# szbonaldo/FedMLP

Measured on AMD Instinct MI355X. Metric: images/sec/client (ICH 224x224 bs=128) at 1/2/4/8 GPUs; mAP vs ref, higher is better.
Workload: dtype f32; 1 GPU; FedMLP stage1 step, Resnet18, ICH-shaped synthetic 3x224x224, C=5, bs=128, one client per GPU, FedAvg all-reduce every 40 steps + once at end; parallelism=clients1, rccl_ranks=1, stream_mode=default: frozen teacher + weight gradients on the engine's side stream, arithmetic=fp32 operands+sums; products as 6 exact bf16 partials on the bf16 matrix pipe

## Files before the change

### fedmlp_amd/_lib.py

```python
import ctypes as C
import os

_HERE = os.path.dirname(os.path.abspath(__file__))
LIB_PATH = os.environ.get("FEDMLP_HIP_LIB") or os.path.join(_HERE, "libfedmlp_hip.so")

FM_MAX_CLASSES = 32
FM_MAX_GROUPS = 8
FM_COMM_ID_BYTES = 128


class FmConfig(C.Structure):
    _fields_ = [("model", C.c_int32), ("n_classes", C.c_int32), ("in_h", C.c_int32),
                ("in_w", C.c_int32), ("max_images", C.c_int32), ("reserved", C.c_int32 * 3),
                ("stream", C.c_void_p)]


class FmAdam(C.Structure):
    _fields_ = [("lr", C.c_float), ("beta1", C.c_float), ("beta2", C.c_float),
                ("eps", C.c_float), ("weight_decay", C.c_float)]


class FmSgd(C.Structure):
    _fields_ = [("lr", C.c_float), ("momentum", C.c_float), ("dampening", C.c_float),
                ("weight_decay", C.c_float), ("nesterov", C.c_int32)]
# ... 17 lines not shown
    "fm_counters": (C.c_int, [_P, _P, _I32]),
    "fm_state_scale": (C.c_int, [_P, C.c_float]),
    "fm_fedavg_fold": (C.c_int, [_P, C.POINTER(_P), _F, _I32, _P]),
    "fm_fed_w": (C.c_int, [_P, C.POINTER(_P), C.POINTER(C.c_double), _I32, _P]),
    "fm_state_dist": (C.c_int, [_P, C.POINTER(_P), _I32, _P, _P, _I32]),
    "fm_stream_mode": (C.c_int, [_P]),
    "fm_mfma_products": (C.c_int, []),
    "fm_products": (C.c_int, [_P]),
    "fm_planes_mode": (C.c_int, [_P]),
    "fm_teacher_snapshot": (C.c_int, [_P]),
    "fm_adam_reset": (C.c_int, [_P, C.POINTER(FmAdam)]),
    "fm_forward_eval": (C.c_int, [_P, _P, _I32, _I32, _P, _P]),
    "fm_step_bce": (C.c_int, [_P, _P, _P, _I32, _F, _I32, _P]),
    "fm_step_stage1": (C.c_int, [_P, _P, _P, _P, _I32, _F, _I32, _I32, _P]),
    "fm_step_stage2": (C.c_int, [_P, _P, _P, _P, _I32, _P]),
    "fm_step_fixmatch": (C.c_int, [_P, _P, _P, _P, _I32, _F, _F, _F, _I32, _I32, _P]),
    "fm_loss_fedlsr": (C.c_int, [_P, _P, _P, _F, C.c_float, C.c_float, _I32, _P, _P]),
    "fm_loss_fedirm_sup": (C.c_int, [_P, _P, _P, _F, _F, _I32, _I32, _I32, _P, _P, _P]),
    "fm_loss_fedirm_rel": (C.c_int, [_P, _P, _P, _P, _F, _F, _I32, _I32, C.c_float, _P, _I32, _P, _P, _P]),
    "fm_step_fedlsr": (C.c_int, [_P, _P, _P, _P, _I32, _F, C.c_float, C.c_float, _P]),
    "fm_loss_rscfed": (C.c_int, [_P, _P, _P, _P, _F, _F, _I32, _I32, _I32, _P, _P]),
    "fm_loss_lakd": (C.c_int, [_P, _P, _P, _P, _F, C.c_float, _I32, _P, _P]),
    "fm_loss_cbafed": (C.c_int, [_P, _P, _P, _F, _I32, _I32, _F, _I32, _P, _P, _P, _P]),
    "fm_step_rscfed": (C.c_int, [_P, _P, _P, _P, _I32, _F, _F, _I32, _I32, C.c_float, C.c_float, _P]),
    "fm_step_fednoro": (C.c_int, [_P, _P, _P, _I32, _F, C.c_float, _P]),
    "fm_step_cbafed": (C.c_int, [_P, _P, _P, _I32, _F, _I32, _I32, _F, _P, _P, _P]),
    "fm_proto_reset": (C.c_int, [_P]),
    "fm_proto_accumulate": (C.c_int, [_P, _P, _P, _P, _I32, _F, _F, C.c_float, C.c_float]),
    "fm_proto_finalize": (C.c_int, [_P, _I32, _I64, _F, _P, _P]),
    "fm_cos_tag": (C.c_int, [_P, _P, _I64, _P, C.POINTER(_I32), _I32, _P]),
    "fm_select_topk": (C.c_int, [_P, _P, _I64, C.c_double, C.c_double, _I32, C.POINTER(_I32),
                                 C.POINTER(_I32), C.POINTER(_I32), C.POINTER(_I32)]),
    "fm_select_topk_rows": (C.c_int, [_P, _P, _I64, _I32, C.POINTER(_I32), C.POINTER(_I32), _I32, C.c_double, C.c_double, _I32,
                                      C.POINTER(_I32), C.POINTER(_I32), C.POINTER(_I32), C.POINTER(_I32)]),
    "fm_augment": (C.c_int, [_P, _P, _P, _P, _I32, _F, _F, _P]),
    "fm_augment_strong": (C.c_int, [_P, _P, _P, _P, _P, _I32, _F, _F, _P]),
    "fm_eval_metrics": (C.c_int, [_P, _P, _P, _I64, _I32, C.c_float, _P, _P, _P]),
    "fm_forward_train": (C.c_int, [_P, _P, _P, _I32, _P, _P]),
    "fm_backward_step": (C.c_int, [_P, _P]),
    "fm_backward_grads": (C.c_int, [_P, _P, _P]),
    "fm_backward_grads_x": (C.c_int, [_P, _P, _P, _P, _P]),
    "fm_forward_recompute": (C.c_int, [_P, _P, _P, _I32]),
    "fm_zero_grad": (C.c_int, [_P]),
    "fm_adam_step": (C.c_int, [_P, C.POINTER(FmAdam)]),
    "fm_get_grads": (C.c_int, [_P, _P]),
    "fm_sgd_reset": (C.c_int, [_P, C.POINTER(FmSgd)]),
    "fm_sgd_step": (C.c_int, [_P, C.POINTER(FmSgd)]),
    "fm_adamw_step": (C.c_int, [_P, C.POINTER(FmAdam)]),
    "fm_set_trainable": (C.c_int, [_P, _P, _I32]),
    "fm_get_trainable": (C.c_int, [_P, _P, _I32]),
    "fm_optim_groups": (C.c_int, [_P, _P, _I32, _I32]),
    "fm_adam_step_groups": (C.c_int, [_P, C.POINTER(FmAdam), _I32]),
    "fm_adamw_step_groups": (C.c_int, [_P, C.POINTER(FmAdam), _I32]),
    "fm_sgd_step_groups": (C.c_int, [_P, C.POINTER(FmSgd), _I32]),
    "fm_grad_norm": (C.c_int, [_P, _P]),
    "fm_clip_grad_norm": (C.c_int, [_P, C.c_float, _P]),
    "fm_clip_grad_value": (C.c_int, [_P, C.c_float]),
    "fm_optim_get_state": (C.c_int, [_P, _P, _P, C.POINTER(_I64)]),
    "fm_optim_set_state": (C.c_int, [_P, _P, _P, _I64]),
    "fm_bn_freeze": (C.c_int, [_P, _I32]),
    "fm_bn_frozen": (C.c_int, [_P]),
    "fm_teacher_axpby": (C.c_int, [_P, C.c_float, C.c_float]),
    "fm_teacher_ema_params": (C.c_int, [_P, C.c_double]),
    "fm_teacher_swap": (C.c_int, [_P]),
    "fm_set_stochastic": (C.c_int, [_P, _P, _P]),
    "fm_feature_dim": (C.c_int, [_P]),
    "fm_profile_enable": (C.c_int, [_P, _I32]),
    "fm_profile_read": (C.c_int, [_P, _I32, C.POINTER(_I64), C.POINTER(C.c_double),
                                  C.POINTER(C.c_double)]),
    "fm_comm_preflight": (C.c_int, []),
    "fm_comm_unique_id": (C.c_int, [C.POINTER(C.c_uint8)]),
    "fm_comm_init": (C.c_int, [_P, C.POINTER(C.c_uint8), _I32, _I32]),
    "fm_comm_destroy": (C.c_int, [_P]),
    "fm_comm_size": (C.c_int, [_P]),
    "fm_fedavg_allreduce": (C.c_int, [_P, C.c_float]),
    "fm_fedavg_tao": (C.c_int, [_P, C.POINTER(C.c_double), C.c_double, _F, C.POINTER(C.c_double)]),
    "fm_fedavg_proto": (C.c_int, [_P, _P, C.c_double, _F, _P]),
    "fm_profile_ops": (C.c_int, [_P, _I32, C.c_char_p, _I32]),
    "fm_debug_num_convs": (C.c_int, [_P]),
    "fm_debug_conv_info": (C.c_int, [_P, _I32, C.POINTER(_I32)]),
    "fm_debug_conv": (C.c_int, [_P, _I32, _I32, _P, _P, _P, _I32, _I32, _P]),
    "fm_debug_conv_fwd": (C.c_int, [_P, _I32, _P, _P, _I32, _I32, _P, _P, _P, _I32, _P, _P, _P, _P]),
    "fm_debug_block_dgrad": (C.c_int, [_P, _I32, _P, _P, _P, _I32]),
    "fm_debug_conv_planes": (C.c_int, [_P, _I32, _P, _I32, _P, _P, _P, _P, _I32, _P, _P]),
    "fm_debug_conv_arm": (C.c_int, [_P, _I32, _I32, _I32]),
    "fm_debug_pw": (C.c_int, [_P, _I32, _I32, _P, _P, _P, _I32, _I32, _P, _P, _P, _P]),
    "fm_debug_pw_fwd": (C.c_int, [_P, _I32, _P, _P, _I32, _I32, _P, _P, _P, _I32, _P, _P, _P, _P]),
    "fm_debug_proj_bwd": (C.c_int, [_P, _I32, _I32, _P, _P, _P, _P, _P, _I32, _I32, _P, _P]),
    "fm_debug_exp_bwd": (C.c_int, [_P, _I32, _P, _P, _P, _P, _P, _I32, _I32, _P, _P]),
    "fm_debug_get_grads": (C.c_int, [_P, _P]),
    "fm_debug_optim_arena": (C.c_int, [_P, _I32, C.POINTER(_P), C.POINTER(_I64)]),
    "fm_debug_entry_spans": (C.c_int, [_P, _P, _I32]),
    "fm_debug_activation": (C.c_int, [_P, _I32, _I32, _I32, _P, C.POINTER(_I32)]),
    "fm_debug_stem_masks": (C.c_int, [_P, _I32, _I32, _P, _P]),
    "fm_debug_lose_part": (C.c_int, [_I32]),
    "fm_debug_lane_delay": (C.c_int, [_P, _I32, _I64, _I32]),
    "fm_debug_lane_points": (C.c_int, [_P, C.POINTER(_I64), _I32]),
    "fm_debug_drop_wait": (C.c_int, [_P, _I32, _I32]),
    "fm_debug_ew": (C.c_int, [_P, _I32, C.POINTER(_P), C.POINTER(_I32), _F]),
    "fm_debug_eff": (C.c_int, [_P, _I32, C.POINTER(_P), C.POINTER(_I32), _F]),
    "fm_debug_eff_ws": (C.c_int, [_I32, C.POINTER(_I32), C.POINTER(C.c_int64)]),
    "fm_debug_head": (C.c_int, [_P, _I32, C.POINTER(_P), C.POINTER(_I32), _F]),
}

ROFL_SYMBOLS = {
    "fm_loss_rofl": (C.c_int, [_P, _P, _P, _P, _P, _I32, _I32, _F, C.c_float, C.c_float, _I32, _P, _P, _I64, _P, _P, _P]),
    "fm_step_rofl": (C.c_int, [_P, _P, _P, _P, _I32, _I32, _F, C.c_float, C.c_float, _I32, _P, _P, _I64, _P]),
}

DRIFT_SYMBOLS = {
    "fm_drift_begin": (C.c_int, [_P, C.c_float, _P, _I32]),
    "fm_drift_last": (C.c_int, [_P, _P]),
    "fm_drift_end": (C.c_int, [_P, _P, C.POINTER(_I64)]),
    "fm_drift_active": (C.c_int, [_P]),
}

_lib = None


def load():
    global _lib
    if _lib is not None:
        return _lib
    if not os.path.exists(LIB_PATH):
        raise RuntimeError(
            f"{LIB_PATH} is missing: the HIP extension is not built and fedmlp_amd has no CPU "
            "fallback. Build it with `make` (or __graft_entry__.build()).")
    import torch
    lib = C.CDLL(LIB_PATH)
    for name, (res, args) in list(SYMBOLS.items()) + list(ROFL_SYMBOLS.items()) + list(DRIFT_SYMBOLS.items()):
        try:
            fn = getattr(lib, name)
        except AttributeError:
            if os.environ.get("FEDMLP_HIP_LIB") and name.startswith("fm_debug_"):
                continue
            raise
        fn.restype = res
        fn.argtypes = args
    _lib = lib
    return lib


class FmError(RuntimeError):
    pass


def check(rc):
    if rc != 0:
        msg = load().fm_last_error()
        raise FmError(f"fedmlp_hip error {rc}: {msg.decode() if msg else ''}")


def fvec(values, n=None):
    vals = [float(v) for v in values]
    if n is not None:
        assert len(vals) == n, (len(vals), n)
    return (C.c_float * len(vals))(*vals)
```

### fedmlp_amd/csrc/common.h

```cpp
#pragma once
#include <hip/hip_runtime.h>
#include <stdint.h>

#include <stdlib.h>

typedef float f32x4 __attribute__((ext_vector_type(4)));

#ifndef FM_F32_FAST_SWISH
#define FM_F32_FAST_SWISH 1
#endif
#ifdef __HIPCC__
__device__ __forceinline__ float fm_swish_f32(float v)
{
#if FM_F32_FAST_SWISH
    return v * __builtin_amdgcn_rcpf(1.f + __expf(-v));
#else
    return v / (1.f + expf(-v));
#endif
}
#endif


#ifndef FM_MFMA_SPLIT_DEFAULT
#define FM_MFMA_SPLIT_DEFAULT 6
// ... 44 lines not shown
{
    if constexpr (NV == 1) st4(p, v[0]);
    else {
        const bf16x4 a = __builtin_convertvector(v[0], bf16x4), b = __builtin_convertvector(v[1], bf16x4);
        *reinterpret_cast<bf16x8*>(p) = __builtin_shufflevector(a, b, 0, 1, 2, 3, 4, 5, 6, 7);
    }
}
template <int NV> __device__ __forceinline__ void ldf(const float* p, f32x4 (&v)[NV])
{
#pragma unroll
    for (int h = 0; h < NV; ++h) v[h] = ld4(p + 4 * h);
}
#endif

#define PCONV_MAX_JOBS 5
struct PconvJob {
    int ntaps;
    unsigned long long tapcode;
    int cib, icc2;
    unsigned wofs, wofs2;
    int Hg, Wg;
    int oh0, ow0;
    int nsteps, k2;
    int npix;
    float rcpHW, rcpW;
    int tilesN;
    int tile0, step0;
};
inline unsigned long long pconv_tapcode(const int* dh, const int* dw, int ntaps)
{
    unsigned long long c = 0;
    for (int t = 0; t < ntaps; ++t) c |= (unsigned long long)(((dh[t] + 1) & 3) | (((dw[t] + 1) & 3) << 2)) << (4 * t);
    return c;
}

struct IgemmParams {
    const float* W;
    const float* X;
    float* Y;
    int dh[9], dw[9];
    int ntaps;
    unsigned long long tapcode;
    int tap_minor;
    int tn_fast;
    int stem_kw, stem_pad;
    int stem_h2;
    int stem3;
    const float* zeros;
    const float* res;
    const float* scale;
    const float* shift;
    float* stats;
    float* slab;
    int* counters;
    long long total_steps;
    int steps_per_block;
    int M, nsteps;
    int Hi, Wi, Ci;
    int Hg, Wg, sg;
    int Ho, Wo, Co;
    int os, oh0, ow0;
    int imgs_per_group;
    int tilesM, tilesN;
    int relu;
    const float* gate = nullptr;
    int gate_HW = 1;
    const float* psc = nullptr;
    const float* psh = nullptr;
    int sp = 0;
    const unsigned short* Wsp = nullptr;
    const unsigned short* Xp = nullptr;
    long long xp_pix = 0;
    unsigned short* Yp = nullptr;
    long long yp_pix = 0;
    const unsigned short* resp = nullptr;
    int wrow = 0;
    int lose_part = 0;
    int* err = nullptr;
    int* err_host = nullptr;
    int njobs = 0;
    PconvJob job[PCONV_MAX_JOBS];
    const unsigned short* Xp2 = nullptr;
    unsigned wsp_bytes = 0;
};
void pconv_debug_lose_part(int on);

struct WgradParams {
    const float* dY;
    const float* X;
    float* slab;
    const int4* tab;
    const float* zeros;
    int M, Nw;
    int Ho, Wo, Hi, Wi, Ci, stride;
    int npix;
    int pix_per_split;
    int tilesM, tilesN;
    int bn;
    int gather_k, gather_pad, gather_kw_p;
    int sp = 0;
};

struct PwgradParams {
    const unsigned short* dYp;
    const unsigned short* Xp;
    float* slab;
    int M, Nw;
    int Ho, Wo, Hi, Wi, Ci, stride, pad, ksz;
    long long npix, xpix;
    int pix_per_split;
    int tilesM, tilesN, nblk_n;
    int sp;
    int nimg, Qtot, q_per_split, splits, xcd_remap;
    unsigned magW, magH;
};
struct StemRowsParams {
    const unsigned short* Xp;
    const unsigned short* Wst;
    float* Y;
    const float* scale;
    const float* shift;
    float* stats;
    int imgs, imgs_per_group, Hp, Wp, Ho, Wo, relu, sp;
    long long plane_bytes;
};
bool stem_rows_takes(int k, int stride, int cout, int hout, int wout, long long plane_bytes);
int stem_rows_stats_tiles(int imgs_per_group, int hout);
void launch_stem_rows(StemRowsParams p, hipStream_t s);
void k_stem_weight_planes(const float* w, unsigned short* dst, int Kw, hipStream_t s);
int launch_pwgrad(PwgradParams p, size_t slab_floats, hipStream_t s);
bool pwgrad_ring_takes(const PwgradParams& p);
int launch_pwgrad_ring(PwgradParams p, size_t slab_floats, hipStream_t s);
bool pwgrad_takes(int M, int Ci, int ksz, long long npix, long long xpix, int Wi, int pad);
void launch_igemm(IgemmParams p, int groups, hipStream_t s);
void launch_pconv(IgemmParams p, int groups, hipStream_t s);
bool pconv_takes(int M, int Ci, long long xp_pix, int Wi);
bool pconv_uses_ts(const IgemmParams& p);
int pconv_tile_m(int M);
int pconv_tile_n(int M);
size_t pconv_slab_floats();
bool launch_conv1x1_stream(const IgemmParams& p, int groups, hipStream_t s);
bool conv1x1_stream_takes(int Ci, int M, int Co);
int igemm_max_blocks();
bool launch_wgrad(const WgradParams& p, int splits, hipStream_t s);
int wgrad_tile_n(int M, int Nw);
int launch_wgrad_skinny(const WgradParams& p, size_t slab_floats, hipStream_t s);
bool wgrad_skinny_takes(const WgradParams& p);
int igemm_tile_n(int M, bool stem = false);
int igemm_tile_m(int M);

#include <stdio.h>
inline void set_max_dyn_lds(const void* fn, int bytes, const char* what)
{
    const hipError_t rc = hipFuncSetAttribute(fn, hipFuncAttributeMaxDynamicSharedMemorySize, bytes);
    if (rc != hipSuccess) fprintf(stderr, "fedmlp_hip: hipFuncSetAttribute(%s, %d B) failed: %s\n", what, bytes, hipGetErrorString(rc));
}
```

### fedmlp_amd/csrc/engine.hip

```cpp
#include <math.h>
#include <stdio.h>
#include <string.h>

#include <algorithm>
#include <string>
#include <unordered_map>
#include <vector>

#include "../../include/fedmlp_hip.h"
#include "../../include/fedmlp_hip_debug.h"
#include "../../include/fedmlp_hip_rofl.h"
#include "../../include/fedmlp_hip_drift.h"
#include "comm.h"
#include "common.h"
#include "kernels.h"
#include "pwconv.h"

static thread_local std::string g_err;
const char* fm_last_error(void) { return g_err.c_str(); }
const char* fm_version(void) { return "fedmlp_hip 0.2 (gfx950)"; }

#define HIPCHK(x)                                                                              \
    do {                                                                                       \
        hipError_t e_ = (x);                                                                   \
// ... 111 lines not shown
    const int32_t* train = nullptr;
};

struct ResGrads { Out dy2, dyd, dy1; };
struct EffGrads { float *dyp = nullptr, *dyd = nullptr, *dye = nullptr, *se_dg = nullptr, *se_dr = nullptr; };

struct StateEntry {
    int kind;
    int conv;
    size_t eng_off;
    size_t n;
    int bn;
    int O = 0, I = 0, KH = 0, KW = 0, Wpad = 0, Ipad = 0;
    int Ostride = 0;
    struct Span { int dense, row; long long len; };
    Span span() const
    {
        if (kind != 0) return {(int)n, (int)n, (long long)n};
        const int dense = KH * Wpad * Ipad, row = Ostride ? Ostride : dense;
        return {dense, row, (long long)(O - 1) * row + dense};
    }
};

struct EvPair { hipEvent_t a, b; int family; double flops; };
struct OpEv { hipEvent_t a, b; int id; };
template <typename J>
struct JobList { J* jobs = nullptr; int n = 0, blocks = 0; };

}

struct fm_engine {
    fm_config cfg;
    Lane main, side;
    Weights student, teacher;
    Acts acts, tacts;
    int C = 0, D = 512, H = 0, W = 0, maxB = 0;
    std::vector<Conv> convs;
    std::vector<Bn> bns;
    std::vector<Block> blocks;
    std::vector<MBConv> mbs;
    int model = 0, c_stem = 0, c_head = -1, bn_stem = 0, bn_head = -1;
    float bn_eps = 1e-5f, bn_mom = 0.1f;
    int maxC = 512;
    ResGrads rg[2];
    EffGrads eg[2];
    float *se_ds = nullptr, *hfeat = nullptr;
    const float *dc_dev = nullptr, *drop_dev = nullptr;
    int pending_views = 0, pending_B = 0;
    float* gacc = nullptr;
    bool gacc_full = false;
    double* norm_part = nullptr;
    float* norm_word = nullptr;
    DistEntry* dist_ent = nullptr;
    DistChunk* dist_chunks = nullptr;
    double* dist_part = nullptr;
    int dist_n_ent = 0, dist_n_chunks = 0;
    uint8_t* strong_ws = nullptr;
    uint8_t* metrics_ws = nullptr;
    size_t metrics_ws_bytes = 0;
    bool bn_freeze = false, pending_fixed = false;
    std::vector<int32_t> trainable, pending_trainable, group_of;
    int n_groups = 0;
    OptChunk* opt_chunks = nullptr;
    int n_opt_chunks = 0;
    std::vector<int> opt_ent;
    std::unordered_map<size_t, int> ent_at;
    std::vector<StateEntry> entries;
    int n_bn_ch = 0;
    size_t NP = 0, NS = 0;
    size_t off_fcw = 0, off_fcb = 0, off_gamma = 0, off_beta = 0, off_rm = 0, off_rv = 0;
    int64_t nf_sd = 0, ni_sd = 0;
    float *grad = nullptr, *adam_m = nullptr, *adam_v = nullptr;
    float* stage_sd = nullptr;
    fm_adam hp{3e-5f, 0.9f, 0.999f, 1e-8f, 5e-4f};
    int64_t adam_t = 0;
    float *x4 = nullptr, *dyh0 = nullptr;
    float* x3 = nullptr;
    bool stem_rows = false;
    unsigned short* x3p = nullptr;
    long long x3p_plane_elems = 0;
    uint8_t* idx0 = nullptr;
    float *GA = nullptr, *GB = nullptr, *GE = nullptr;
    float *ws_stats = nullptr, *ws_part = nullptr;
    int stats_conv = -1, stats_tiles_n = 0;
    size_t slab_floats = 0;
    float *ca = nullptr, *cb = nullptr, *cc = nullptr;
    float *feat = nullptr, *logits = nullptr, *tfeat = nullptr, *tlogits = nullptr, *dlogits = nullptr;
    float* psum = nullptr;
    int64_t *pcnt = nullptr, *tcnt = nullptr;
    float* zeros = nullptr;
    int *sel_counts = nullptr, *sel_top = nullptr, *sel_bot = nullptr, *cls_dev = nullptr;
    int sel_cap = 0;
    double *rofl_rowloss = nullptr, *rofl_dist = nullptr;
    float* rofl_cos = nullptr;
    int* rofl_keep = nullptr;
    bool drift_on = false, drift_shifted = false, drift_track = false;
    float drift_mu = 0.f;
    int64_t drift_steps = 0;
    float *drift_anchor = nullptr, *drift_shift = nullptr, *drift_gsum = nullptr, *drift_gcorr = nullptr;
    int* tag_buf = nullptr;
    size_t tag_buf_ints = 0;
    bool prof = false, prof_fail = false;
    hipError_t soft_err = hipSuccess;
    int* dev_err = nullptr;
    int* host_err = nullptr;
    int* host_err_dev = nullptr;
    bool oprof = false;
    int ctx = -1;
    std::vector<std::string> op_names;
    std::vector<double> op_ms;
    std::vector<int64_t> op_n;
    std::vector<OpEv> opevs;
    std::vector<EvPair> evs;
    std::vector<hipEvent_t> ev_free;
    double prof_ms[FM_PROFILE_FAMILIES] = {}, prof_flops[FM_PROFILE_FAMILIES] = {};
    int64_t prof_n[FM_PROFILE_FAMILIES] = {};
    std::vector<void*> allocs;
    JobList<PackJob> pack_jobs;
    unsigned short* wpl_d = nullptr;
    bool dgrad_dirty = true;
    float* stem_dpack = nullptr;
    bool stem_dpack_stale = true;
    JobList<SplitJob> split_f, split_d;
    bool planes = false;
    unsigned short* xp_scratch = nullptr;
    unsigned short* xp_scratch2 = nullptr;
    size_t xp_scratch_elems = 0;
    const float* xp_scratch_src = nullptr;
    long long xp_scratch_npix = 0;
    void* comm = nullptr;
    int comm_rank = 0, comm_world = 0;
    double* comm_buf = nullptr;
    size_t comm_buf_n = 0;
    int precision = 0;
    int products = 6;
    int stream_mode = 0;
    int dt = DT_F32;
    size_t wb_numel = 0;
    JobList<CastJob> cast_jobs;
    bool fuse_gate = false;
    hipEvent_t ev_in = nullptr, ev_t = nullptr;
    bool side_ok = false;
    int in_img0 = 0;
    bool side_w = false;
    hipEvent_t ev_p[4][2] = {}, ev_c[4][2] = {}, ev_wdone = nullptr;
    float* stem_col = nullptr;
    struct LaneDbg {
        bool armed = false, fired = false;
        int lane = 0, micros = 0;
        int64_t at = 0, ticks = 0;
        int64_t points[2] = {0, 0};
        uint32_t drop = 0;
        int64_t waits[FM_WAIT_KINDS] = {}, skipped[FM_WAIT_KINDS] = {};
    } ldbg;
};
static void lane_point_armed(fm_engine* e, int lane);
static inline void lane_point(fm_engine* e, int lane)
{
    if (e->ldbg.armed) lane_point_armed(e, lane);
}
static inline hipError_t lane_wait(fm_engine* e, int kind, hipStream_t st, hipEvent_t ev)
{
    fm_engine::LaneDbg& d = e->ldbg;
    d.waits[kind] += 1;
    if (d.drop >> kind & 1) { d.skipped[kind] += 1; return hipSuccess; }
    return hipStreamWaitEvent(st, ev, 0);
// ... 496 lines not shown
    e->side_ok = true;
    if (e->stream_mode != 0) return FM_OK;
    DALLOC(s.ws_slab, e->slab_floats);
    if (e->model == 0) {
        const Conv& c0 = e->convs[0];
        const size_t pooled = B * (c0.hout / 2) * (c0.wout / 2) * 64;
        ResGrads& g = e->rg[1];
        DALLOC(g.dy2.f, pooled); DALLOC(g.dyd.f, pooled); DALLOC(g.dy1.f, pooled);
        if (e->planes) { PALLOC(g.dy2.p, pooled); PALLOC(g.dyd.p, pooled); PALLOC(g.dy1.p, pooled); }
    } else {
        const EffSizes z = eff_sizes(e);
        EffGrads& g = e->eg[1];
        AALLOC(g.dyp, z.t_small); AALLOC(g.dyd, z.t_mid); AALLOC(g.dye, z.t_big);
        DALLOC(g.se_dg, B * z.max_ce); DALLOC(g.se_dr, B * z.max_cs);
    }
    for (int k = 0; k < 4; ++k)
        for (int q = 0; q < 2; ++q) {
            HIPCHK(hipEventCreateWithFlags(&e->ev_p[k][q], hipEventDisableTiming));
            HIPCHK(hipEventCreateWithFlags(&e->ev_c[k][q], hipEventDisableTiming));
        }
    HIPCHK(hipEventCreateWithFlags(&e->ev_wdone, hipEventDisableTiming));
    e->side_w = true;
    return FM_OK;
}

int alloc_workspaces(fm_engine* e)
{
    const size_t B = e->maxB;
    for (Weights* w : {&e->student, &e->teacher}) {
        DALLOC(w->state, e->NS);
        HIPCHK(hipMemset(w->state, 0, e->NS * 4));
        DALLOC(w->ev_scale, e->n_bn_ch); DALLOC(w->ev_shift, e->n_bn_ch);
    }
    DALLOC(e->grad, e->NP); DALLOC(e->adam_m, e->NP); DALLOC(e->adam_v, e->NP);
    HIPCHK(hipMemset(e->grad, 0, e->NP * 4));
    HIPCHK(hipMemset(e->adam_m, 0, e->NP * 4)); HIPCHK(hipMemset(e->adam_v, 0, e->NP * 4));
    DALLOC(e->stage_sd, (size_t)e->nf_sd);
    DALLOC(e->x4, B * e->H * e->W * 4);
    if (e->convs[0].stem3) {
        const size_t n3 = B * e->convs[0].Hp * e->convs[0].Wp * 3 + 64;
        DALLOC(e->x3, n3);
        HIPCHK(hipMemset(e->x3, 0, n3 * 4));
        const Conv& c0 = e->convs[0];
        e->x3p_plane_elems = (long long)B * c0.Hp * c0.Wp * 4;
        e->stem_rows = e->planes && stem_rows_takes(c0.k, c0.stride, c0.cout_p, c0.hout, c0.wout, e->x3p_plane_elems * 2);
        if (e->stem_rows) {
            DALLOC(e->x3p, (size_t)3 * e->x3p_plane_elems + 64);
            HIPCHK(hipMemset(e->x3p, 0, ((size_t)3 * e->x3p_plane_elems + 64) * 2));
            DALLOC(e->student.wst, 7 * 3 * 64 * 32); DALLOC(e->teacher.wst, 7 * 3 * 64 * 32);
        }
    }
    size_t max_stats = 0, max_slab = 0;
    for (auto& c : e->convs) {
        AALLOC(c.y, B * c.hout * c.wout * c.cout_p);
        if (c.cin == 3 && e->precision) AALLOC(e->stem_col, B * c.hout * c.wout * c.Kw);
        size_t tiles = (B * c.hout * c.wout + igemm_tile_n(c.cout_p, c.cin == 3) - 1) / igemm_tile_n(c.cout_p, c.cin == 3) + 2;
        if (e->precision) tiles = std::max<size_t>(tiles, B * c.hout * c.wout / 128 + 4);
        max_stats = std::max(max_stats, (tiles + 2 * 32) * 2 * c.cout_p);
        max_slab = std::max(max_slab, c.w_numel);
    }
    for (auto& b : e->bns) {
        DALLOC(b.mean, 2 * b.C); DALLOC(b.istd, 2 * b.C); DALLOC(b.scale, 2 * b.C); DALLOC(b.shift, 2 * b.C);
    }
    RCCHK(alloc_acts(e, e->acts, false));
    bool side = e->stream_mode != 1;
    const Conv& c0 = e->convs[0];
    if (e->model == 0) {
        const size_t pooled = B * (c0.hout / 2) * (c0.wout / 2) * 64;
        DALLOC(e->idx0, pooled);
        DALLOC(e->dyh0, B * c0.hout * c0.wout * 64);
        ResGrads& g = e->rg[0];
        DALLOC(e->GA, pooled); DALLOC(g.dy2.f, pooled); DALLOC(g.dyd.f, pooled); DALLOC(g.dy1.f, pooled); DALLOC(e->GE, pooled);
    } else {
        const EffSizes z = eff_sizes(e);
        AALLOC(e->GA, z.g_io); AALLOC(e->GB, z.g_io);
        EffGrads& g = e->eg[0];
        g.dyd = e->acts.T_mid;
        AALLOC(g.dyp, z.t_small); AALLOC(g.dye, z.t_big);
        DALLOC(g.se_dg, B * z.max_ce); DALLOC(g.se_dr, B * z.max_cs); DALLOC(e->se_ds, B * z.max_ce);
        side = side && side_fits(e);
        DALLOC(e->hfeat, B * e->D);
    }
    DALLOC(e->ws_stats, max_stats);
    DALLOC(e->ws_part, (size_t)2 * (1024 + 32) * 2 * e->maxC);
    e->slab_floats = std::max<size_t>(max_slab * 8, (size_t)48 << 20);
    DALLOC(e->main.ws_slab, e->slab_floats);
    e->main.rec = e->main.ws_slab;
    DALLOC(e->ca, 2 * e->maxC); DALLOC(e->cb, 2 * e->maxC); DALLOC(e->cc, 2 * e->maxC);
    DALLOC(e->feat, B * e->D); DALLOC(e->tfeat, B * e->D);
    DALLOC(e->logits, B * e->C); DALLOC(e->tlogits, B * e->C); DALLOC(e->dlogits, B * e->C);
    DALLOC(e->psum, (size_t)2 * e->C * e->D); DALLOC(e->pcnt, 2 * e->C); DALLOC(e->tcnt, e->C);
    DALLOC(e->sel_counts, 2); DALLOC(e->cls_dev, FM_MAX_CLASSES);
    DALLOC(e->zeros, 64);
    if (e->planes) {
        const size_t pooled = B * (c0.hout / 2) * (c0.wout / 2) * 64;
        PALLOC(e->rg[0].dy2.p, pooled); PALLOC(e->rg[0].dyd.p, pooled); PALLOC(e->rg[0].dy1.p, pooled);
        size_t mx = 0;
        for (auto& c : e->convs) {
            if (c.cin == 3) continue;
            mx = std::max(mx, std::max(B * c.hin * c.win * c.cin_p, B * c.hout * c.wout * c.cout_p));
        }
        e->xp_scratch_elems = mx * 3;
        float* t3 = nullptr;
        DALLOC(t3, (e->xp_scratch_elems + 1) / 2);
        e->xp_scratch = reinterpret_cast<unsigned short*>(t3);
        DALLOC(t3, (e->xp_scratch_elems + 1) / 2);
        e->xp_scratch2 = reinterpret_cast<unsigned short*>(t3);
    }
    DALLOC(e->main.sk_slab, sk_floats());
    DALLOC(e->dev_err, 16);
    HIPCHK(hipMemset(e->dev_err, 0, 16 * sizeof(int)));
    HIPCHK(hipHostMalloc(reinterpret_cast<void**>(&e->host_err), 64, hipHostMallocMapped));
    *e->host_err = 0;
    HIPCHK(hipHostGetDevicePointer(reinterpret_cast<void**>(&e->host_err_dev), e->host_err, 0));
    DALLOC(e->main.sk_counters, (size_t)1 << 20);
    HIPCHK(hipMemset(e->main.sk_counters, 0, ((size_t)1 << 20) * 4));
    HIPCHK(hipMemset(e->zeros, 0, 64 * 4));
    if (e->model == 0) side = side && side_fits(e);
    e->rg[1] = e->rg[0]; e->eg[1] = e->eg[0];
    return side ? alloc_side(e) : FM_OK;
}

hipEvent_t get_ev(fm_engine* e)
{
    if (!e->ev_free.empty()) { hipEvent_t v = e->ev_free.back(); e->ev_free.pop_back(); return v; }
    hipEvent_t v = nullptr;
    if (hipEventCreate(&v) != hipSuccess) { e->prof_fail = true; return nullptr; }
    return v;
}
struct ProfScope {
    fm_engine* e; hipStream_t st; hipEvent_t a{}, b{}; int fam; double fl; bool on;
    ProfScope(fm_engine* e_, const Lane& L, int family, double flops) : e(e_), st(L.st), fam(family), fl(flops), on(e_->prof)
    {
        if (on) {
            a = get_ev(e); b = get_ev(e);
            on = a && b;
            if (on && hipEventRecord(a, st) != hipSuccess) { e->prof_fail = true; on = false; }
        }
    }
    ~ProfScope()
    {
        if (on) {
            if (hipEventRecord(b, st) != hipSuccess) e->prof_fail = true;
            e->evs.push_back({a, b, fam, fl});
        }
    }
};

struct OpScope {
    fm_engine* e; hipStream_t st; hipEvent_t a{}, b{}; int id = -1; bool on;
    OpScope(fm_engine* e_, const Lane& L, const char* op) : e(e_), st(L.st), on(e_->oprof)
    {
        lane_point(e_, &L == &e_->side);
        if (!on) return;
        char lab[96];
        snprintf(lab, sizeof lab, "%s@%d", op, e->ctx);
        for (size_t i = 0; i < e->op_names.size(); ++i)
            if (e->op_names[i] == lab) { id = (int)i; break; }
        if (id < 0) { id = (int)e->op_names.size(); e->op_names.push_back(lab); e->op_ms.push_back(0); e->op_n.push_back(0); }
        a = get_ev(e); b = get_ev(e);
        on = a && b && hipEventRecord(a, st) == hipSuccess;
    }
    ~OpScope()
    {
        if (on && hipEventRecord(b, st) == hipSuccess) e->opevs.push_back({a, b, id});
    }
};
// ... 142 lines not shown
    const Epilogue& ep = o.epi;
    const Prologue& pro = o.pro;
    float* const stats = o.stats;
    const Arm arm = fwd_arm(e, c, imgs);
    const int tiles_n = stats_tiles_for(arm, c, imgs / groups, groups, pro.gate != nullptr);
    if (stats) { e->stats_conv = ci; e->stats_tiles_n = tiles_n; }
    const int fam = prof_family(arm, c.cout_p);
    const double flops = 2.0 * c.macs_per_img * imgs;
    switch (arm) {
    case Arm::StemRows: {
        StemRowsParams q{};
        q.Xp = e->x3p + (size_t)e->in_img0 * c.Hp * c.Wp * 4; q.Wst = W.wst; q.Y = y.f;
        q.scale = ep.scale; q.shift = ep.shift; q.stats = stats; q.relu = ep.act;
        q.imgs = imgs; q.imgs_per_group = imgs / groups; q.Hp = c.Hp; q.Wp = c.Wp; q.Ho = c.hout; q.Wo = c.wout;
        q.sp = e->products; q.plane_bytes = e->x3p_plane_elems * 2;
        ProfScope ps(e, L, fam, flops);
        launch_stem_rows(q, L.st);
        return;
    }
    case Arm::PwConv: {
        const bool stem16 = c.cin == 3;
        PwParams q{};
        q.zeros = e->zeros;
        q.W = W.wb + c.wb_off;
        q.X = reinterpret_cast<const bf16*>(stem16 ? e->stem_col : x.f); q.Y = reinterpret_cast<bf16*>(y.f);
        if (stem16) q.X += (size_t)e->in_img0 * c.hout * c.wout * c.Kw;
        q.M = c.cout_p; q.K = stem16 ? c.Kw : c.cin_p;
        q.npix = (imgs / groups) * c.hout * c.wout; q.groups = groups;
        q.scale = ep.scale; q.shift = ep.shift; q.res = reinterpret_cast<const bf16*>(ep.res.f); q.act = ep.act;
        q.stats = stats;
        if (pro.gate) { q.psc = pro.psc; q.psh = pro.psh; q.gate = pro.gate; }
        q.HW = c.hout * c.wout;
        launch_pw_conv(q, L.st);
        return;
    }
    case Arm::PconvTs: case Arm::PconvTap: case Arm::Igemm: case Arm::IgemmStem: break;
    default: soft(e, hipErrorInvalidValue); return;
    }
    IgemmParams p{};
    p.Y = y.f; p.slab = L.sk_slab; p.counters = L.sk_counters; p.err = e->dev_err; p.err_host = e->host_err_dev; p.sp = e->products;
    conv_fwd_geometry(c, p);
    p.res = ep.res.f; p.scale = ep.scale; p.shift = ep.shift; p.stats = stats;
    p.Ho = c.hout; p.Wo = c.wout; p.Co = c.cout_p;
    p.os = 1; p.oh0 = 0; p.ow0 = 0;
    p.imgs_per_group = imgs / groups;
    p.tilesN = tiles_n;
    p.relu = ep.act;
    if (arm == Arm::PconvTs || arm == Arm::PconvTap) {
        p.xp_pix = (long long)imgs * c.hin * c.win;
        p.Xp = x.p ? x.p : scratch_planes(e, L, x.f, p.xp_pix, c.cin_p);
        p.Wsp = W.wpl_f + c.pl_off;
        p.Yp = y.p; p.yp_pix = (long long)imgs * c.hout * c.wout; p.resp = ep.res.p;
        p.tilesM = c.cout_p / pconv_tile_m(c.cout_p);
        ProfScope ps(e, L, fam, flops);
        launch_pconv(p, groups, L.st);
        return;
    }
    p.W = W.state + c.w_off; p.X = x.f; p.zeros = e->zeros; p.nsteps = c.nsteps;
    if (!e->planes && c.pl_off >= 0) p.Wsp = W.wpl_f + c.pl_off;
    if (c.cin == 3) {
        p.stem_kw = c.k; p.stem_pad = c.pad; p.stem_h2 = c.kw_p == 8 ? 1 : 0; p.stem3 = c.stem3 ? 1 : 0;
        if (c.stem3) p.X = e->x3 + (size_t)e->in_img0 * c.Hp * c.Wp * 3;
        else p.X = x.f + (size_t)e->in_img0 * c.hin * c.win * 4;
    }
    if (c.stem3) { p.Hi = c.Hp; p.Wi = c.Wp; }
    if (pro.gate) {
        p.gate = pro.gate; p.gate_HW = c.hout * c.wout; p.psc = pro.psc; p.psh = pro.psh;
        if (!conv1x1_stream_takes(c.cin_p, c.cout_p, c.cout_p) || c.k != 1 || c.stride != 1 || (pro.psc && !stats) ||
            (!pro.psc && stats))
            soft(e, hipErrorInvalidValue);
    }
    p.tilesM = (c.cout_p + igemm_tile_m(c.cout_p) - 1) / igemm_tile_m(c.cout_p);
    ProfScope ps(e, L, fam, flops);
    launch_igemm(p, groups, L.st);
}

int stats_tiles(fm_engine* e, int ci)
{
    if (e->stats_conv != ci) soft(e, hipErrorInvalidValue);
    return e->stats_tiles_n;
}

struct DgradAdd { const float* res = nullptr; bool acc_cls0 = false; };
void conv_dgrad(fm_engine* e, Lane& L, int ci, In dy, float* dx, int imgs, const DgradAdd& add = {})
{
    Conv& c = e->convs[ci];
    const Arm arm = dgrad_arm(e, c, imgs);
    const long long xp_pix = (long long)imgs * c.hout * c.wout;
    switch (arm) {
    case Arm::PwConv: {
        PwParams q{};
        q.zeros = e->zeros;
        q.W = e->student.wb + c.wbt_off;
        q.X = reinterpret_cast<const bf16*>(dy.f); q.Y = reinterpret_cast<bf16*>(dx);
        q.M = c.cin_p; q.K = c.cout_p;
        q.npix = imgs * c.hout * c.wout; q.groups = 1;
        q.res = reinterpret_cast<const bf16*>(add.res);
        q.HW = c.hout * c.wout;
        launch_pw_conv(q, L.st);
        return;
    }
    case Arm::PconvTs: case Arm::PconvTap: case Arm::Igemm: break;
    default: soft(e, hipErrorInvalidValue); return;
    }
    const bool planes = arm != Arm::Igemm;
    if (planes && !dy.p) dy.p = scratch_planes(e, L, dy.f, xp_pix, c.cout_p);
    for (int k = 0; k < c.ncls; ++k) {
        DgradClass& d = c.cls[k];
        IgemmParams p{};
        p.Y = dx; p.slab = L.sk_slab; p.counters = L.sk_counters; p.err = e->dev_err; p.err_host = e->host_err_dev; p.sp = e->products;
        conv_dgrad_geometry(c, d, p);
        p.res = add.res ? add.res : ((add.acc_cls0 && d.ph == 0 && d.pw == 0) ? dx : nullptr);
        p.Ho = c.hin; p.Wo = c.win; p.Co = c.cin_p;
        p.os = c.stride; p.oh0 = d.ph; p.ow0 = d.pw;
        p.imgs_per_group = imgs;
        p.relu = 0;
        const int bn = planes ? pconv_tile_n(c.cin_p) : igemm_tile_n(c.cin_p);
        p.tilesN = (imgs * p.Hg * p.Wg + bn - 1) / bn;
        const double flops = 2.0 * c.macs_per_img * imgs * d.taps.n / (double)(c.k * c.k);
        if (planes) {
            p.Xp = dy.p; p.xp_pix = xp_pix; p.Wsp = e->wpl_d + d.pl_off;
            p.tilesM = c.cin_p / pconv_tile_m(c.cin_p);
            ProfScope ps(e, L, prof_family(pconv_arm(p), c.cin_p), flops);
            launch_pconv(p, 1, L.st);
        } else {
            p.W = d.wpack; p.X = dy.f; p.zeros = e->zeros; p.nsteps = d.nsteps;
            if (!e->planes && d.pl_off >= 0) p.Wsp = e->wpl_d + d.pl_off;
            p.tilesM = (c.cin_p + igemm_tile_m(c.cin_p) - 1) / igemm_tile_m(c.cin_p);
            ProfScope ps(e, L, prof_family(arm, c.cin_p), flops);
            launch_igemm(p, 1, L.st);
        }
    }
}

bool block_dgrad(fm_engine* e, Lane& L, int c1i, int dsi, In dy1, In dyd, float* dx, int imgs)
{
    Conv& c = e->convs[c1i];
    Conv& d = e->convs[dsi];
    const long long xp_pix = (long long)imgs * c.hout * c.wout;
    if (c.ncls != 4 || d.ncls != 1 || !dgrad_uses_pconv(e, c, imgs) || d.cls[0].pl_off < 0) return false;
    static_assert(PCONV_MAX_JOBS >= 4, "one job per parity class");
    const DgradClass& d0 = d.cls[0];
    if (c.stride != 2 || d.stride != 2 || d.k != 1 || d.cin_p != c.cin_p || d.cout_p != c.cout_p || d.hin != c.hin || d.win != c.win ||
        d.hout != c.hout || d.wout != c.wout || d0.ph != 0 || d0.pw != 0 || d0.dh[0] != 0 || d0.dw[0] != 0)
        return false;
    const DgradClass& c0 = c.cls[0];
    if (c0.ph != 0 || c0.pw != 0 || c0.taps.n != 1 || c0.dh[0] != 0 || c0.dw[0] != 0) return false;
    if (!dy1.p) dy1.p = scratch_planes(e, L, dy1.f, xp_pix, c.cout_p);
    if (!dyd.p) {
        if ((size_t)xp_pix * d.cout_p * 3 > e->xp_scratch_elems) { soft(e, hipErrorInvalidValue); return true; }
        k_split_planes(dyd.f, e->xp_scratch2, xp_pix, d.cout_p, L.st);
        dyd.p = e->xp_scratch2;
    }
    if (!dy1.p) return true;
    IgemmParams p{};
    p.Xp = dy1.p; p.Xp2 = dyd.p; p.xp_pix = xp_pix; p.Wsp = e->wpl_d;
    p.Y = dx; p.slab = L.sk_slab; p.counters = L.sk_counters; p.err = e->dev_err; p.err_host = e->host_err_dev; p.sp = e->products;
    p.M = c.cin_p;
    p.Hi = c.hout; p.Wi = c.wout; p.Ci = c.cout_p;
    p.sg = 1;
    p.Ho = c.hin; p.Wo = c.win; p.Co = c.cin_p;
    p.os = c.stride;
    p.imgs_per_group = imgs;
    p.tilesM = c.cin_p / pconv_tile_m(c.cin_p);
    p.relu = 0;
    p.njobs = c.ncls;
    for (int k = 0; k < c.ncls; ++k) {
        const DgradClass& q = c.cls[k];
        PconvJob& j = p.job[k];
        j.ntaps = q.taps.n; j.tapcode = pconv_tapcode(q.dh, q.dw, q.taps.n);
        j.cib = j.icc2 = c.cout_p >> 5;
        j.wofs = j.wofs2 = (unsigned)(q.pl_off * 2);
        j.Hg = (c.hin - q.ph + c.stride - 1) / c.stride;
        j.Wg = (c.win - q.pw + c.stride - 1) / c.stride;
        j.oh0 = q.ph; j.ow0 = q.pw;
    }
    p.job[0].cib += d.cout_p >> 5;
    p.job[0].wofs2 = (unsigned)(d0.pl_off * 2);
    ProfScope ps(e, L, prof_family(Arm::PconvTap, c.cin_p), 2.0 * (c.macs_per_img + d.macs_per_img) * imgs);
    launch_pconv(p, 1, L.st);
    return true;
}

void conv_wgrad(fm_engine* e, Lane& L, int ci, In x, In dy, int imgs, const Prologue& pro = {}, int pix_per_group = 0)
{
    const Conv& c = e->convs[ci];
    const Arm arm = wgrad_arm(e, c, imgs);
    const int fam = prof_family(arm, c.cout_p);
    const double flops = 2.0 * c.macs_per_img * imgs;
    int sk = 0;
    switch (arm) {
    case Arm::Pwgrad:
    case Arm::PwgradRing: {
        PwgradParams q{};
        pwgrad_geometry(e, c, imgs, q);
        if (!x.p) x.p = scratch_planes(e, L, x.f, q.xpix, c.cin_p);
        if (!dy.p) {
            if ((size_t)q.npix * c.cout_p * 3 > e->xp_scratch_elems) { soft(e, hipErrorInvalidValue); return; }
            k_split_planes(dy.f, e->xp_scratch2, q.npix, c.cout_p, L.st);
            dy.p = e->xp_scratch2;
        }
        q.dYp = dy.p; q.Xp = x.p; q.slab = L.ws_slab;
        ProfScope ps(e, L, fam, flops);
        sk = arm == Arm::PwgradRing ? launch_pwgrad_ring(q, e->slab_floats, L.st) : launch_pwgrad(q, e->slab_floats, L.st);
        if (sk <= 0) soft(e, hipErrorInvalidValue);
        break;
    }
// ... 17 lines not shown
        if (c.stem3) p.X = e->x3;
        ProfScope ps(e, L, fam, flops);
        if (arm == Arm::WgradSkinny) {
            sk = launch_wgrad_skinny(p, e->slab_floats, L.st);
            if (sk <= 0) soft(e, hipErrorInvalidValue);
            break;
        }
        const int bm = c.cout_p >= 128 ? 128 : 64, bn = wgrad_tile_n(c.cout_p, c.Kw);
        p.bn = bn;
        p.tilesM = (c.cout_p + bm - 1) / bm;
        p.tilesN = (c.Kw + bn - 1) / bn;
        const int tiles = p.tilesM * p.tilesN;
        constexpr int WG_SLOTS = 512;
        int splits = std::max(1, WG_SLOTS / tiles);
        const int max_by_pix = std::max(1, p.npix / 256);
        const int max_by_mem = (int)std::max<size_t>(1, e->slab_floats / c.w_numel);
        splits = std::max(1, std::min(splits, std::min(max_by_pix, max_by_mem)));
        p.pix_per_split = (((p.npix + splits - 1) / splits) + 31) & ~31;
        sk = (p.npix + p.pix_per_split - 1) / p.pix_per_split;
        if (!launch_wgrad(p, sk, L.st)) soft(e, hipErrorInvalidValue);
        break;
    }
    default: soft(e, hipErrorInvalidValue); return;
    }
    if (sk > 0) k_reduce_slabs(L.ws_slab, e->grad + c.w_off, sk, (int64_t)c.w_numel, L.st);
    if (c.stem3) k_stem3_mask_grad(e->grad + c.w_off, c.cout_p, L.st);
}

struct BnSlots { float *gamma, *beta, *run_mean, *run_var, *dgamma, *dbeta; };
BnSlots bn_slots(const fm_engine* e, const Bn& b)
{
    float *S = e->student.state + b.ch_off, *G = e->grad + b.ch_off;
    return {S + e->off_gamma, S + e->off_beta, S + e->off_rm, S + e->off_rv, G + e->off_gamma, G + e->off_beta};
}

void bn_fwd_fixed(fm_engine* e, Lane& L, Bn& b, int groups)
{
    const BnSlots s = bn_slots(e, b);
    k_bn_finalize_frozen(groups, b.C, s.gamma, s.beta, s.run_mean, s.run_var, b.mean, b.istd, b.scale, b.shift, e->bn_eps, L.st, e->dev_err);
}
void bn_fwd_stats(fm_engine* e, Lane& L, int bi, const float* part, int groups, int tiles, int count, BnMode mode, const int* skip)
{
    Bn& b = e->bns[bi];
    if (mode == BnMode::Frozen) { bn_fwd_fixed(e, L, b, groups); return; }
    const BnSlots s = bn_slots(e, b);
    const bool run = mode == BnMode::Batch;
    k_bn_finalize(part, groups, tiles, b.C, count, s.gamma, s.beta, run ? s.run_mean : nullptr, run ? s.run_var : nullptr, b.mean, b.istd,
                  b.scale, b.shift, e->bn_eps, e->bn_mom, L.st, skip);
    if (run) e->student.counters[bi] += groups;
}
void bn_fwd_finalize(fm_engine* e, Lane& L, int ci, int groups, int imgs_per_group, BnMode mode)
{
    const Conv& c = e->convs[ci];
    const int tiles = mode == BnMode::Frozen ? 0 : stats_tiles(e, ci);
    bn_fwd_stats(e, L, c.bn, e->ws_stats, groups, tiles, imgs_per_group * c.hout * c.wout, mode, e->dev_err);
}

void conv_fwd_train(fm_engine* e, Lane& L, int ci, const Weights& W, In x, int groups, int B, BnMode mode, const char* op = nullptr,
                    const Prologue& pro = {})
{
    const Out y{e->convs[ci].y};
    const FwdOps o{.stats = e->ws_stats, .pro = pro};
    if (op) {
        { OP(L, op); conv_fwd(e, L, ci, W, x, y, groups * B, groups, o); }
        { OP(L, "bn_fwd_finalize"); bn_fwd_finalize(e, L, ci, groups, B, mode); }
    } else {
        LP(L); conv_fwd(e, L, ci, W, x, y, groups * B, groups, o);
        LP(L); bn_fwd_finalize(e, L, ci, groups, B, mode);
    }
}
void conv_fwd_eval(fm_engine* e, Lane& L, int ci, const Weights& W, In x, Out y, int imgs, int act, In res = {}, const Prologue& pro = {})
{
    const int ch = e->bns[e->convs[ci].bn].ch_off;
    conv_fwd(e, L, ci, W, x, y, imgs, 1, {.pro = pro, .epi = {W.ev_scale + ch, W.ev_shift + ch, res, act}});
}

void bn_bwd_finalize(fm_engine* e, Lane& L, const Bn& b, int groups, int partials, int count, bool frozen)
{
    const BnSlots s = bn_slots(e, b);
    k_bn_bwd_finalize(e->ws_part, groups, partials, b.C, count, s.gamma, b.mean, b.istd, e->ca, e->cb, e->cc, s.dgamma, s.dbeta, L.st, frozen);
}
enum class Mask { None, Z, ZPlane, OwnOutput };
void bn_bwd(fm_engine* e, Lane& L, int bi, const float* dz, Out dy, int groups, int imgs_per_group, bool frozen, Mask mask = Mask::None,
            In z = {}, float* dyh_out = nullptr)
{
    const Conv& c = e->convs[bi];
    Bn& b = e->bns[bi];
    const int pix = imgs_per_group * c.hout * c.wout;
    const char* fy = getenv("FM_BN_MASK_FROM_Y");
    const int from_y = fy ? atoi(fy) : 1;
    const float *msc = nullptr, *msh = nullptr, *zf = nullptr;
    const unsigned short* zh = nullptr;
    if (mask == Mask::Z || (mask == Mask::OwnOutput && !from_y && z.f)) zf = z.f;
    else if (mask == Mask::ZPlane) zh = z.p;
    else if (mask == Mask::OwnOutput) { msc = b.scale; msh = b.shift; }
    k_bn_bwd_reduce(dz, zf, c.y, b.mean, b.istd, e->ws_part, groups, pix, b.C, L.st, msc, msh, zh);
    bn_bwd_finalize(e, L, b, groups, bn_bwd_blocks(pix), pix, frozen);
    if (dy.p) k_bn_bwd_apply_planes(dz, zf, c.y, e->ca, e->cb, e->cc, dy.f, dy.p, dyh_out, groups, pix, b.C, L.st, msc, msh, zh);
    else k_bn_bwd_apply(dz, zf, c.y, e->ca, e->cb, e->cc, dy.f, dyh_out, groups, pix, b.C, L.st, msc, msh);
}

void to_nhwc4(fm_engine* e, Lane& L, const float* const* xs, int groups, int B)
{
    if (e->precision && e->model == 1) {
        const Conv& c = e->convs[e->c_stem];
        for (int g = 0; g < groups; ++g)
            k_stem_im2col(xs[g], reinterpret_cast<bf16*>(e->stem_col) + (size_t)g * B * c.hout * c.wout * c.Kw, B, e->H, e->W, c.hout,
                          c.wout, c.k, c.stride, c.pad, c.pad, L.st);
        return;
    }
    if (e->convs[0].stem3) {
        const Conv& c = e->convs[0];
        for (int g = 0; g < groups; ++g)
            k_frame_nhwc3(xs[g], e->x3 + (size_t)g * B * c.Hp * c.Wp * 3, B, e->H, e->W, c.Hp, c.Wp, 3, 3, 0, L.st,
                          e->stem_rows ? e->x3p + (size_t)g * B * c.Hp * c.Wp * 4 : nullptr, e->x3p_plane_elems);
        return;
    }
    for (int g = 0; g < groups; ++g)
        k_nchw_to_nhwc4(xs[g], e->x4 + (size_t)g * B * e->H * e->W * 4, B, e->H, e->W, L.st);
}

void student_copies_stale(fm_engine* e)
{
    e->dgrad_dirty = true;
    e->stem_dpack_stale = true;
}
enum class Moved { Weights, Stats };
void net_changed(fm_engine* e, Weights& W, Moved what = Moved::Weights)
{
    W.ev_dirty = true;
    if (what == Moved::Stats) return;
    W.fwd_dirty = true;
    if (&W == &e->student) student_copies_stale(e);
}
void ensure_eval_affine(fm_engine* e, Lane& L, Weights& W)
{
    if (!W.ev_dirty) return;
    const float* S = W.state;
    k_bn_eval_affine(S + e->off_gamma, S + e->off_beta, S + e->off_rm, S + e->off_rv, W.ev_scale, W.ev_shift, e->n_bn_ch, e->bn_eps, L.st);
    W.ev_dirty = false;
}
void ensure_fwd_shadows(fm_engine* e, Weights& W)
{
    if (!W.fwd_dirty) return;
    Lane& L = e->main;
    if (e->precision) launch_cast_weights(W.state, W.wb, e->cast_jobs.jobs, e->cast_jobs.n, e->cast_jobs.blocks, L.st);
    else if (e->planes) {
        k_split_weights_bm(W.state, W.wpl_f, e->split_f.jobs, e->split_f.n, e->split_f.blocks, L.st);
        if (e->stem_rows) k_stem_weight_planes(W.state + e->convs[0].w_off, W.wst, e->convs[0].Kw, L.st);
    } else
        k_split_weights(W.state, W.wpl_f, e->split_f.jobs, e->split_f.n, e->split_f.blocks, L.st);
    W.fwd_dirty = false;
}
void ensure_packed(fm_engine* e)
{
    ensure_fwd_shadows(e, e->student);
    if (!e->dgrad_dirty) return;
    Lane& L = e->main;
    if (!e->precision && e->pack_jobs.n)
        k_pack_dgrad_all(e->student.state, e->pack_jobs.jobs, e->pack_jobs.n, e->pack_jobs.blocks, L.st);
    (e->planes ? k_split_weights_bm : k_split_weights)(nullptr, e->wpl_d, e->split_d.jobs, e->split_d.n, e->split_d.blocks, L.st);
    e->dgrad_dirty = false;
}

void forward_train(fm_engine* e, Lane& L, Acts& A, int groups, int B, BnMode mode)
{
    const int imgs = groups * B;
    const Weights& W = e->student;
    const float* S = W.state;
    Conv& c0 = e->convs[0];
    conv_fwd_train(e, L, 0, W, {e->x4}, groups, B, mode);
    LP(L);
    if (A.p0.p) k_stem_pool_planes(c0.y, e->bns[0].scale, e->bns[0].shift, A.p0.f, e->idx0, A.p0.p, groups, B, c0.hout, c0.wout, 64, L.st);
    else k_stem_pool(c0.y, e->bns[0].scale, e->bns[0].shift, A.p0.f, e->idx0, groups, B, c0.hout, c0.wout, 64, L.st);
    auto apply = [&](int ci, Out out, In res = {}, int ds = -1) {
        const Conv& c = e->convs[ci];
        const Bn& b = e->bns[ci];
        const float* y2 = ds >= 0 ? e->convs[ds].y : nullptr;
        const float *s2 = y2 ? e->bns[ds].scale : nullptr, *h2 = y2 ? e->bns[ds].shift : nullptr;
        const int pix = B * c.hout * c.wout;
// ... 220 lines not shown
inline bool conv_on(const fm_engine* e, const int32_t* tr, int ci) { return ent_on(e, tr, e->convs[ci].w_off); }
inline bool bn_on(const fm_engine* e, const int32_t* tr, int bi)
{
    return ent_on(e, tr, e->off_gamma + e->bns[bi].ch_off) || ent_on(e, tr, e->off_beta + e->bns[bi].ch_off);
}
OptSel group_sel(const fm_engine* e)
{
    OptSel sel{};
    for (size_t i = 0; i < e->entries.size(); ++i) {
        const int t = e->opt_ent[i];
        if (t < 0) continue;
        const int g = e->group_of[i];
        const bool on = g >= 0 && (e->trainable.empty() || e->trainable[i] != 0);
        opt_sel_set(sel, t, on ? (unsigned)g : OPT_SKIP);
    }
    return sel;
}
OptSel mask_sel(const fm_engine* e, const int32_t* tr)
{
    OptSel sel{};
    for (size_t i = 0; i < e->entries.size(); ++i)
        if (e->opt_ent[i] >= 0) opt_sel_set(sel, e->opt_ent[i], tr[i] != 0 ? 0u : 1u);
    return sel;
}
void adam_step_groups(fm_engine* e, const fm_adam* hp, int n)
{
    const float* g = drift_grad(e, e->gacc);
    e->adam_t += 1;
    OptAdamArgs a{};
    for (int i = 0; i < n; ++i) a.hp[i] = adam_hp(hp[i], e->adam_t);
    k_adam_groups(e->student.state, g, e->adam_m, e->adam_v, e->opt_chunks, e->n_opt_chunks, group_sel(e), a, e->main.st, e->dev_err);
    weights_stepped(e);
}
void adamw_step_groups(fm_engine* e, const fm_adam* hp, int n)
{
    const float* g = drift_grad(e, e->gacc);
    e->adam_t += 1;
    OptAdamWArgs a{};
    for (int i = 0; i < n; ++i) a.hp[i] = adamw_hp(hp[i], e->adam_t);
    k_adamw_groups(e->student.state, g, e->adam_m, e->adam_v, e->opt_chunks, e->n_opt_chunks, group_sel(e), a, e->main.st, e->dev_err);
    weights_stepped(e);
}
void sgd_step_groups(fm_engine* e, const fm_sgd* hp, int n)
{
    const float* g = drift_grad(e, e->gacc);
    const bool first = e->adam_t == 0;
    e->adam_t += 1;
    OptSgdArgs a{};
    for (int i = 0; i < n; ++i) a.hp[i] = sgd_hp(hp[i], first);
    k_sgd_groups(e->student.state, g, e->adam_m, e->opt_chunks, e->n_opt_chunks, group_sel(e), a, e->main.st, e->dev_err);
    weights_stepped(e);
}

Lane& side_begin(fm_engine* e, int k, int par)
{
    if (!e->side_w) return e->main;
    soft(e, hipEventRecord(e->ev_p[k][par], e->main.st));
    soft(e, lane_wait(e, FM_WAIT_SIDE_BEGIN, e->side.st, e->ev_p[k][par]));
    return e->side;
}
void side_end(fm_engine* e, int k, int par)
{
    if (e->side_w) soft(e, hipEventRecord(e->ev_c[k][par], e->side.st));
}
void side_guard(fm_engine* e, int k, int par)
{
    if (e->side_w) soft(e, lane_wait(e, FM_WAIT_SIDE_GUARD, e->main.st, e->ev_c[k][par]));
}
void side_join(fm_engine* e)
{
    if (!e->side_w) return;
    soft(e, hipEventRecord(e->ev_wdone, e->side.st));
    soft(e, lane_wait(e, FM_WAIT_SIDE_JOIN, e->main.st, e->ev_wdone));
}
template <typename Launch>
void side_wgrad(fm_engine* e, bool& forked, int k, int par, const char* op, Launch&& launch)
{
    forked = true;
    Lane& SL = side_begin(e, k, par);
    { OP(SL, op); launch(SL); }
    side_end(e, k, par);
}

void backward_and_step(fm_engine* e, int groups, int B, const Bwd& bw)
{
    const int imgs = groups * B;
    Lane& L = e->main;
    const Acts& A = e->acts;
    const float* S = e->student.state;
    const Conv& cl = e->convs[e->blocks.back().c2];
    const int32_t* tr = bw.train;
    const int nb = (int)e->blocks.size();
    int first = 0;
    if (tr && !(bw.dx[0] || bw.dx[1])) {
        auto blk_live = [&](const Block& k) {
            return conv_on(e, tr, k.c1) || bn_on(e, tr, k.c1) || conv_on(e, tr, k.c2) || bn_on(e, tr, k.c2) ||
                   (k.ds >= 0 && (conv_on(e, tr, k.ds) || bn_on(e, tr, k.ds)));
        };
        first = nb + 2;
        if (ent_on(e, tr, e->off_fcw) || ent_on(e, tr, e->off_fcb)) first = nb + 1;
        for (int b = nb - 1; b >= 0; --b)
            if (blk_live(e->blocks[b])) first = 1 + b;
        if (conv_on(e, tr, 0) || bn_on(e, tr, 0)) first = 0;
    }
    bool forked = false;
    if (first > nb + 1) return;
    e->ctx = 500;
    { OP(L, "k_fc_bwd"); k_fc_bwd(e->dlogits, e->feat, S + e->off_fcw, nullptr, e->grad + e->off_fcw, e->grad + e->off_fcb, e->GA, DT_F32, imgs,
             512, e->C, cl.hout * cl.wout, L.st, bw.dfeat); }
    float *ga = e->GA, *ge = e->GE;
    for (int b = nb - 1; b >= 0 && 1 + b >= first; --b) {
        const Block& blk = e->blocks[b];
        e->ctx = 400 + b;
        const BlockActs& a = A.blk[b];
        const int par = b & 1;
        const ResGrads& g = e->rg[par];
        const Out dy2 = kept(g.dy2), dyd = kept(g.dyd), dy1 = kept(g.dy1);
        const In in = b == 0 ? In(A.p0) : In(A.blk[b - 1].out);
        const bool last = b + 1 == (int)e->blocks.size();
        const In zo = last ? In{a.out.f} : In(kept(a.out));
        side_guard(e, 0, par);
        { OP(L, "bn_bwd"); bn_bwd(e, L, blk.c2, ga, dy2, groups, B, bw.frozen, zo.f ? Mask::Z : Mask::ZPlane, zo, ga); }
        if (blk.ds >= 0) { side_guard(e, 1, par); OP(L, "bn_bwd"); bn_bwd(e, L, blk.ds, ga, dyd, groups, B, bw.frozen); }
        side_guard(e, 2, par);
        { OP(L, "conv_dgrad"); conv_dgrad(e, L, blk.c2, dy2, g.dy1.f, imgs); }
        if (conv_on(e, tr, blk.c2))
            side_wgrad(e, forked, 0, par, "conv_wgrad", [&](Lane& SL) { conv_wgrad(e, SL, blk.c2, kept(a.z1), dy2, imgs); });
        { OP(L, "bn_bwd"); bn_bwd(e, L, blk.c1, g.dy1.f, dy1, groups, B, bw.frozen, Mask::OwnOutput, kept(a.z1)); }
        { OP(L, "conv_dgrad");
          if (blk.ds < 0) conv_dgrad(e, L, blk.c1, dy1, ge, imgs, {.res = ga});
          else if (!block_dgrad(e, L, blk.c1, blk.ds, dy1, dyd, ge, imgs)) {
              conv_dgrad(e, L, blk.ds, dyd, ge, imgs);
              conv_dgrad(e, L, blk.c1, dy1, ge, imgs, {.acc_cls0 = true});
          } }
        if (conv_on(e, tr, blk.c1))
            side_wgrad(e, forked, 2, par, "conv_wgrad", [&](Lane& SL) { conv_wgrad(e, SL, blk.c1, in, dy1, imgs); });
        if (blk.ds >= 0 && conv_on(e, tr, blk.ds))
            side_wgrad(e, forked, 1, par, "conv_wgrad", [&](Lane& SL) { conv_wgrad(e, SL, blk.ds, in, dyd, imgs); });
        std::swap(ga, ge);
    }
    const Conv& c0 = e->convs[0];
    e->ctx = 399;
    if (first == 0) {
        OP(L, "stem_pool_bn_bwd");
        Bn& b0 = e->bns[0];
        const BnSlots s0 = bn_slots(e, b0);
        const int pooled_pg = B * (c0.hout / 2) * (c0.wout / 2), pix = B * c0.hout * c0.wout;
        k_stem_pool_bn_reduce(ga, A.p0.f, e->idx0, c0.y, b0.mean, b0.istd, e->ws_part, groups, B, c0.hout, c0.wout, 64, L.st, s0.gamma,
                              s0.beta);
        bn_bwd_finalize(e, L, b0, groups, stem_pool_bn_blocks(pooled_pg), pix, bw.frozen);
        k_stem_pool_bn_apply(ga, A.p0.f, e->idx0, c0.y, e->ca, e->cb, e->cc, e->dyh0, groups, B, c0.hout, c0.wout, 64, L.st);
    }
    if (first == 0) {
        if (bw.dx[0] || bw.dx[1]) { OP(L, "stem_dgrad"); stem_dgrad_views(e, L, e->dyh0, groups, B, bw.dx); }
        if (conv_on(e, tr, 0)) { OP(L, "conv_wgrad"); conv_wgrad(e, L, 0, {e->x4}, {e->dyh0}, imgs); }
    }
    if (forked) side_join(e);
    if (bw.step) adam_step(e, e->grad);
}

bool fuse_for(fm_engine* e, const MBConv& m)
{
    if (e->precision) return e->fuse_gate && pw_tiles_m(m.cout_p, m.ce_p) <= 2;
    return pw_proj_bwd_f32_nch(m.ce_p, m.cout_p, 1, m.hout * m.wout) > 0 && conv1x1_stream_takes(m.ce_p, m.cout_p, m.cout_p);
}

void bn_fwd_tensor(fm_engine* e, Lane& L, int bi, const float* y, int groups, int pix_per_group, int HW, BnMode mode, int partials)
{
    if (!partials && mode != BnMode::Frozen)
        k_chan_reduce(nullptr, e->dt, y, e->dt, nullptr, nullptr, nullptr, nullptr, nullptr, e->ws_part, groups, pix_per_group,
                      HW, e->bns[bi].C, 0, 0, nullptr, nullptr, L.st);
    bn_fwd_stats(e, L, bi, e->ws_part, groups, partials ? partials : bn_bwd_blocks(pix_per_group), pix_per_group, mode, nullptr);
}

struct BnActOps { const float *rowscale = nullptr, *gate = nullptr, *dsv = nullptr; int partials = 0; };
void bnact_bwd(fm_engine* e, Lane& L, int bi, const float* dz, const float* y, float* dy, int groups, int pix_per_group, int HW, int act,
               bool frozen, const BnActOps& o = {})
{
    Bn& b = e->bns[bi];
    if (!o.partials)
        k_chan_reduce(dz, e->dt, y, e->dt, b.mean, b.istd, b.scale, b.shift, o.rowscale, e->ws_part, groups, pix_per_group, HW, b.C,
                      1, act, o.gate, o.dsv, L.st);
    bn_bwd_finalize(e, L, b, groups, o.partials ? o.partials : bn_bwd_blocks(pix_per_group), pix_per_group, frozen);
    k_bnact_bwd_apply(dz, e->dt, y, e->dt, e->ca, e->cb, e->cc, b.scale, b.shift, o.rowscale, dy, groups, pix_per_group, HW,
                      b.C, act, o.gate, o.dsv, L.st);
}

void eff_forward_train(fm_engine* e, Lane& L, Acts& A, int groups, int B, BnMode mode)
{
    const int imgs = groups * B;
    const Weights& W = e->student;
    const float* S = W.state;
    Conv& cs = e->convs[e->c_stem];
    e->ctx = -1;
    conv_fwd_train(e, L, e->c_stem, W, {e->x4}, groups, B, mode, "conv_fwd");
    {
        Bn& b = e->bns[e->bn_stem];
        { OP(L, "k_bnact_apply"); k_bnact_apply(cs.y, e->dt, b.scale, b.shift, nullptr, nullptr, A.a0, e->dt, groups, B * cs.hout * cs.wout,
                      cs.hout * cs.wout, b.C, 2, L.st); }
    }
    const float* cur = A.a0;
    for (size_t i = 0; i < e->mbs.size(); ++i) {
        const MBConv& m = e->mbs[i];
        MBActs& a = A.mb[i];
        e->ctx = (int)i;
        const int HWi = m.hin * m.win, HWo = m.hout * m.wout;
        const float* a_e = cur;
        if (m.c_exp >= 0) {
            Conv& ce = e->convs[m.c_exp];
            conv_fwd_train(e, L, m.c_exp, W, {cur}, groups, B, mode, "exp_fwd");
            Bn& b = e->bns[m.bn0];
// ... 1748 lines not shown
    ARGCHK(imgs >= 1 && imgs <= e->maxB && groups >= 1 && groups <= 2 && imgs % groups == 0, "imgs/groups");
    Conv& c = e->convs[conv];
    ensure_packed(e);
    const float* bn = bn_dev;
    const size_t gl = (size_t)groups * c.cout_p;
    const BnCoef coef{bn + 3 * gl, bn + 4 * gl, nullptr, nullptr, bn, bn + gl, bn + 2 * gl};
    const int sk = launch_exp_bwd(e, e->main, c, da_dev, ye_dev, x_dev, res_dev, dx_dev, coef, imgs, groups);
    ARGCHK(sk > 0, "shape not handled by the fused expand backward");
    k_reduce_slabs(e->main.ws_slab, dw_dev, sk, (int64_t)c.w_numel, e->main.st);
    HIPCHK(hipGetLastError());
    return FM_OK;
}

int fm_debug_optim_arena(fm_engine* e, int32_t which, float** dev_ptr, int64_t* numel)
{
    ARGCHK(e && dev_ptr && numel && which >= 0 && which <= 3, "null / which");
    if (which == 2 && !e->gacc) {
        DALLOC(e->gacc, e->NP);
        HIPCHK(hipMemsetAsync(e->gacc, 0, e->NP * 4, e->main.st));
    }
    *dev_ptr = which == 0 ? e->adam_m : (which == 1 ? e->adam_v : (which == 2 ? e->gacc : e->grad));
    *numel = (int64_t)e->NP;
    return FM_OK;
}

int fm_debug_entry_spans(fm_engine* e, int64_t* off_len, int32_t n_entries)
{
    ARGCHK(e && off_len && n_entries == (int32_t)e->entries.size(), "null / entry count");
    RCCHK(ensure_opt_table(e));
    std::vector<OptChunk> chunks;
    std::vector<int> ent;
    std::unordered_map<size_t, int> at;
    build_opt_table(e->entries, e->NP, chunks, ent, at);
    for (int32_t i = 0; i < n_entries; ++i) { off_len[2 * i] = -1; off_len[2 * i + 1] = 0; }
    std::vector<int> of_table(chunks.empty() ? 0 : chunks.back().ent + 1, -1);
    for (int32_t i = 0; i < n_entries; ++i)
        if (ent[i] >= 0) of_table[ent[i]] = i;
    for (const OptChunk& c : chunks) {
        const int i = of_table[c.ent];
        if (off_len[2 * i] < 0) off_len[2 * i] = c.begin;
        off_len[2 * i + 1] += c.len;
    }
    return FM_OK;
}

int fm_debug_get_grads(fm_engine* e, float* host_f32)
{
    ARGCHK(e && host_f32, "null");
    RCCHK(arena_to_state_dict(e, e->grad, e->stage_sd, true));
    HIPCHK(hipMemcpyAsync(host_f32, e->stage_sd, (size_t)e->nf_sd * 4, hipMemcpyDeviceToHost, e->main.st));
    HIPCHK(hipStreamSynchronize(e->main.st));
    return FM_OK;
}

int fm_profile_ops(fm_engine* e, int32_t enable, char* buf, int32_t cap)
{
    ARGCHK(e, "null engine");
    HIPCHK(hipStreamSynchronize(e->main.st));
    for (auto& p : e->opevs) {
        float t = 0.f;
        if (hipEventElapsedTime(&t, p.a, p.b) == hipSuccess) { e->op_ms[p.id] += t; e->op_n[p.id] += 1; }
        e->ev_free.push_back(p.a); e->ev_free.push_back(p.b);
    }
    e->opevs.clear();
    if (buf && cap > 0) {
        std::string out;
        char line[160];
        for (size_t i = 0; i < e->op_names.size(); ++i) {
            snprintf(line, sizeof line, "%s\t%lld\t%.6f\n", e->op_names[i].c_str(), (long long)e->op_n[i], e->op_ms[i]);
            out += line;
        }
        snprintf(buf, (size_t)cap, "%s", out.c_str());
        e->op_names.clear(); e->op_ms.clear(); e->op_n.clear();
    }
    e->oprof = enable != 0;
    return FM_OK;
}

int fm_debug_num_convs(fm_engine* e) { return e ? (int)e->convs.size() : 0; }

int fm_debug_activation(fm_engine* e, int32_t kind, int32_t block, int32_t imgs, float* host_nhwc, int32_t* dims4)
{
    ARGCHK(e && dims4 && e->model == 0, "ResNet-18 engine only");
    ARGCHK(block >= 0 && block < (int)e->blocks.size() && (kind == 0 || kind == 1), "kind/block");
    ARGCHK(imgs >= 1 && imgs <= e->maxB, "imgs");
    const Out t = kind == 0 ? e->acts.blk[block].z1 : e->acts.blk[block].out;
    const Conv& c = e->convs[e->blocks[block].c1];
    dims4[0] = imgs; dims4[1] = c.hout; dims4[2] = c.wout; dims4[3] = c.cout;
    if (host_nhwc) {
        if (e->planes && (kind == 0 || block + 1 < (int)e->blocks.size()))
            k_planes_to_f32(t.p, t.f, (long long)imgs * c.hout * c.wout, c.cout, e->main.st);
        HIPCHK(hipMemcpyAsync(host_nhwc, t.f, (size_t)imgs * c.hout * c.wout * c.cout * 4,
                              hipMemcpyDeviceToHost, e->main.st));
        HIPCHK(hipStreamSynchronize(e->main.st));
    }
    return FM_OK;
}

int fm_debug_lose_part(int32_t on)
{
    pconv_debug_lose_part(on);
    return FM_OK;
}

static void lane_point_armed(fm_engine* e, int lane)
{
    fm_engine::LaneDbg& d = e->ldbg;
    const int64_t pos = d.points[lane]++;
    if (d.fired || lane != d.lane || pos != d.at || d.micros <= 0) return;
    d.fired = true;
    k_lane_delay(d.ticks, 3 * d.micros, lane ? e->side.st : e->main.st);
}

int fm_debug_lane_delay(fm_engine* e, int32_t lane, int64_t at, int32_t micros)
{
    ARGCHK(e, "null engine");
    ARGCHK(lane == 0 || lane == 1, "fm_debug_lane_delay: lane is 0 (main) or 1 (side)");
    ARGCHK(lane == 0 || e->side_ok, "fm_debug_lane_delay: lane 1 on a handle without a side stream");
    ARGCHK(at >= 0, "fm_debug_lane_delay: at >= 0");
    ARGCHK(micros >= 0 && micros <= FM_LANE_DELAY_MAX_US, "fm_debug_lane_delay: 0 <= micros <= FM_LANE_DELAY_MAX_US");
    int dev = 0, khz = 0;
    if (hipGetDevice(&dev) != hipSuccess || hipDeviceGetAttribute(&khz, hipDeviceAttributeWallClockRate, dev) != hipSuccess || khz <= 0)
        khz = 100000;
    fm_engine::LaneDbg& d = e->ldbg;
    const uint32_t drop = d.drop;
    d = fm_engine::LaneDbg{};
    d.drop = drop;
    d.armed = true;
    d.lane = lane; d.at = at; d.micros = micros;
    d.ticks = (int64_t)micros * khz / 1000;
    return FM_OK;
}

int fm_debug_lane_points(fm_engine* e, int64_t* out16, int32_t disarm)
{
    ARGCHK(e && out16, "null");
    fm_engine::LaneDbg& d = e->ldbg;
    for (int i = 0; i < 16; ++i) out16[i] = 0;
    out16[0] = d.points[0]; out16[1] = d.points[1]; out16[2] = d.fired;
    for (int k = 0; k < FM_WAIT_KINDS; ++k) { out16[3 + k] = d.waits[k]; out16[3 + FM_WAIT_KINDS + k] = d.skipped[k]; }
    if (disarm) d.armed = false;
    return FM_OK;
}

int fm_debug_drop_wait(fm_engine* e, int32_t which, int32_t on)
{
    ARGCHK(e, "null engine");
    ARGCHK(which >= 0 && which < FM_WAIT_KINDS, "fm_debug_drop_wait: unknown wait kind");
    if (on) e->ldbg.drop |= 1u << which;
    else e->ldbg.drop &= ~(1u << which);
    return FM_OK;
}

int fm_debug_stem_masks(fm_engine* e, int32_t imgs, int32_t groups, uint8_t* relu_bits_host, uint8_t* argmax_host)
{
    ARGCHK(e && e->model == 0 && !e->precision, "ResNet-18 engine only");
    ARGCHK(imgs >= 1 && imgs <= e->maxB && groups >= 1 && imgs % groups == 0, "imgs / groups");
    const Conv& c0 = e->convs[0];
    const int64_t pix = (int64_t)imgs * c0.hout * c0.wout;
    if (relu_bits_host) {
        uint8_t* bits = nullptr;
        HIPCHK(hipMalloc(&bits, (size_t)pix * 8));
        k_stem_relu_bits(e->acts.stem_y, e->bns[0].scale, e->bns[0].shift, bits, groups, pix / groups, 64, e->main.st);
        hipError_t rc = hipMemcpyAsync(relu_bits_host, bits, (size_t)pix * 8, hipMemcpyDeviceToHost, e->main.st);
        if (rc == hipSuccess) rc = hipStreamSynchronize(e->main.st);
        (void)hipFree(bits);
        HIPCHK(rc);
    }
    if (argmax_host) {
        HIPCHK(hipMemcpyAsync(argmax_host, e->idx0, (size_t)imgs * (c0.hout / 2) * (c0.wout / 2) * 64, hipMemcpyDeviceToHost, e->main.st));
        HIPCHK(hipStreamSynchronize(e->main.st));
    }
    return FM_OK;
}

int fm_debug_block_dgrad(fm_engine* e, int32_t block, const float* dy1_dev, const float* dyd_dev, float* dx_dev, int32_t imgs)
{
    ARGCHK(e && dy1_dev && dyd_dev && dx_dev, "null tensor");
    ARGCHK(e->model == 0 && !e->precision, "fm_debug_block_dgrad: a precision-0 ResNet-18 engine");
    ARGCHK(block >= 0 && block < (int)e->blocks.size() && e->blocks[block].ds >= 0, "block has no downsample");
    ARGCHK(imgs >= 1 && imgs <= e->maxB, "imgs");
    ensure_packed(e);
    const Block& blk = e->blocks[block];
    if (!block_dgrad(e, e->main, blk.c1, blk.ds, {dy1_dev}, {dyd_dev}, dx_dev, imgs)) {
        conv_dgrad(e, e->main, blk.ds, {dyd_dev}, dx_dev, imgs);
        conv_dgrad(e, e->main, blk.c1, {dy1_dev}, dx_dev, imgs, {.acc_cls0 = true});
    }
    return FM_OK;
}

int fm_debug_conv_info(fm_engine* e, int32_t conv, int32_t* info16)
{
    ARGCHK(e && info16 && conv >= 0 && conv < (int)e->convs.size(), "conv index");
    const Conv& c = e->convs[conv];
    const int v[16] = {c.cin, c.cout, c.k, c.stride, c.pad, c.hin, c.win, c.hout, c.wout, c.cin_p, c.Kw, c.kw_p,
                       c.cout_p, 0, 0, 0};
    memcpy(info16, v, sizeof v);
    return FM_OK;
}

int fm_debug_conv(fm_engine* e, int32_t op, int32_t conv, const float* x_dev, const float* dy_dev, float* out_dev,
                  int32_t imgs, int32_t groups, float* stats_dev)
{
    ARGCHK(e && out_dev && conv >= 0 && conv < (int)e->convs.size(), "conv index");
    ARGCHK(!e->precision, "fm_debug_conv works on fp32 tensors: create the engine with precision 0");
    ARGCHK(imgs >= 1 && imgs <= e->maxB && groups >= 1 && imgs % groups == 0, "imgs/groups");
    Conv& c = e->convs[conv];
    if (c.stem3 && x_dev)
        k_frame_nhwc3(x_dev, e->x3, imgs, c.hin, c.win, c.Hp, c.Wp, 3, 3, 1, e->main.st, e->stem_rows ? e->x3p : nullptr, e->x3p_plane_elems);
    ensure_packed(e);
    if (op == 0) {
        ARGCHK(x_dev, "x");
        conv_fwd(e, e->main, conv, e->student, {x_dev}, {out_dev}, imgs, groups, {.stats = stats_dev ? e->ws_stats : nullptr});
        if (stats_dev) RCCHK(debug_fold_stats(e, conv, groups, stats_dev));
    } else if (op == 1) {
        ARGCHK(dy_dev && (c.ncls > 0 || c.cin == 3), "dgrad unavailable for this conv");
        ensure_packed(e);
        if (c.cin == 3) {
            RCCHK(ensure_stem_dpack(e));
            stem_dgrad(e, e->main, dy_dev, out_dev, imgs, true);
        } else conv_dgrad(e, e->main, conv, {dy_dev}, out_dev, imgs);
    } else if (op == 2) {
        ARGCHK(x_dev && dy_dev, "x/dy");
        conv_wgrad(e, e->main, conv, {x_dev}, {dy_dev}, imgs);
        HIPCHK(hipMemcpyAsync(out_dev, e->grad + c.w_off, c.w_numel * 4, hipMemcpyDeviceToDevice, e->main.st));
    } else {
        ARGCHK(false, "op");
    }
    return FM_OK;
}

int fm_debug_conv_fwd(fm_engine* e, int32_t conv, const float* x_dev, float* out_dev, int32_t imgs, int32_t groups,
                      const float* scale_dev, const float* shift_dev, const float* res_dev, int32_t act, const float* psc_dev,
                      const float* psh_dev, const float* gate_dev, float* stats_dev)
{
    ARGCHK(e && x_dev && out_dev && conv >= 0 && conv < (int)e->convs.size(), "conv index");
    ARGCHK(!e->precision, "fm_debug_conv_fwd works on fp32 tensors: create the engine with precision 0");
    ARGCHK(imgs >= 1 && imgs <= e->maxB && groups >= 1 && imgs % groups == 0, "imgs/groups");
    ARGCHK(act >= 0 && act <= 2, "act");
    Conv& c = e->convs[conv];
    ARGCHK(!scale_dev == !shift_dev, "scale and shift come together");
    ARGCHK(!psc_dev == !psh_dev, "psc and psh come together");
    const bool epi = scale_dev != nullptr, pro = gate_dev != nullptr;
    ARGCHK(epi || (!res_dev && act == 0), "res / act belong to the eval epilogue: give scale and shift");
    ARGCHK(!epi || (!stats_dev && groups == 1), "the eval epilogue runs without statistics on one group");
    ARGCHK(!(c.cin == 3 && res_dev), "no graph hands a stem a residual (the stem_rows kernel has no such operand)");
    ARGCHK(pro || !psc_dev, "psc / psh without a gate");
    if (pro) {
        ARGCHK(e->model == 1 && c.k == 1 && c.stride == 1 && conv1x1_stream_takes(c.cin_p, c.cout_p, c.cout_p),
               "an operand prologue needs a 1x1 convolution of an EfficientNet handle that streams through conv1x1.hip");
        ARGCHK(psc_dev ? (stats_dev && !epi) : !stats_dev,
               "prologue forms: gate alone without statistics, or psc + psh + gate with statistics and no epilogue");
    }
    if (e->planes && c.cin != 3)
        ARGCHK(conv_uses_pconv(e, c, imgs) && (size_t)imgs * c.hin * c.win * c.cin_p * 3 <= e->xp_scratch_elems,
               "shape outside the planes kernel");
    if (c.stem3)
        k_frame_nhwc3(x_dev, e->x3, imgs, c.hin, c.win, c.Hp, c.Wp, 3, 3, 1, e->main.st, e->stem_rows ? e->x3p : nullptr, e->x3p_plane_elems);
    ensure_packed(e);
    const Prologue pr{psc_dev, psh_dev, gate_dev};
    conv_fwd(e, e->main, conv, e->student, {x_dev}, {out_dev}, imgs, groups,
             {stats_dev ? e->ws_stats : nullptr, pr, {scale_dev, shift_dev, {res_dev}, act}});
    if (stats_dev) RCCHK(debug_fold_stats(e, conv, groups, stats_dev));
    HIPCHK(hipGetLastError());
    return FM_OK;
}

int fm_debug_conv_planes(fm_engine* e, int32_t conv, const uint16_t* xp_dev, int32_t imgs, const float* scale_dev,
                         const float* shift_dev, const float* res_dev, const uint16_t* resp_dev, int32_t relu, float* out_dev,
                         uint16_t* outp_dev)
{
// ... 367 lines not shown
```

### fedmlp_amd/csrc/pconv.hip

```cpp
#include <stdlib.h>

#include <algorithm>
#include <type_traits>

#include "common.h"
#include "kernels.h"
#include "split3.h"

#if __HIP_DEVICE_COMPILE__
template <int IMM> __device__ __forceinline__ sp_u32x4 pc_lds_read128(unsigned addr)
{
    sp_u32x4 v;
    asm volatile("ds_read_b128 %0, %1 offset:%2" : "=v"(v) : "v"(addr), "n"(IMM));
    return v;
}
__device__ __forceinline__ void pc_divmod(int x, int d, float rcp, int& q, int& r)
{
    q = (int)((float)x * rcp);
    r = x - q * d;
    if (r < 0) { --q; r += d; }
    else if (r >= d) { ++q; r -= d; }
}
template <int CTRL> __device__ __forceinline__ float pc_dpp(float v)
{
    return __builtin_bit_cast(float, __builtin_amdgcn_update_dpp(0, __builtin_bit_cast(int, v), CTRL, 0xF, 0xF, false));
}
template <typename F> __device__ __forceinline__ void pc_for4(F f)
{
    f(std::integral_constant<int, 0>{}); f(std::integral_constant<int, 1>{});
    f(std::integral_constant<int, 2>{}); f(std::integral_constant<int, 3>{});
}
template <int SP> __device__ __forceinline__ f32x4 pc_mfma(const sp_u32x4 (&a)[3], const sp_u32x4 (&b)[3], f32x4 v)
{
    return mfma_split<SP>(a[0], a[1], a[2], b[0], b[1], b[2], v);
}
#endif

#ifdef PC_PHASES
__device__ unsigned long long pc_prof[256 * 8];
#define PC_T(i) do { const unsigned long long t_ = clock64(); pc_acc[i] += t_ - pc_t; pc_t = t_; } while (0)
#else
#define PC_T(i) do { } while (0)
#endif
#ifndef PC_WAVES_PER_EU
#define PC_WAVES_PER_EU 2
#endif
template <int FR, int FC, int NS, int SP, bool TS = false>
__global__ __launch_bounds__(512, PC_WAVES_PER_EU) void pconv_kernel(const IgemmParams p)
{
#if __HIP_DEVICE_COMPILE__
#ifdef PC_PHASES
    unsigned long long pc_acc[8] = {0, 0, 0, 0, 0, 0, 0, 0};
    unsigned long long pc_t = clock64();
#endif
    constexpr int WN = 4;
    constexpr int BM = 32 * FR, BN = 64 * FC;
    constexpr int GA = BM / 16, GB = TS ? (BN + 2 + 15) / 16 : BN / 16;
    constexpr int BROWS = 16 * GB;
    constexpr int SA = 3 * BM * 64, SB = 3 * BROWS * 64;
    constexpr int NSB = TS ? 2 : NS;
    static_assert(!TS || FC == 4, "tap-row sharing: 256-pixel tiles");
    constexpr int JA = (3 * GA + 7) / 8;
    constexpr int RGB = (GB + 7) / 8;
    static_assert(NS == 2 && FC == 4 && (FR == 2 || FR == 4), "two LDS stages, 256-pixel tiles, 64 or 128 rows");
    typedef __attribute__((address_space(3))) void lds_void;
    extern __shared__ __attribute__((aligned(16))) unsigned char smem[];
    const int tid = threadIdx.x;
    const int lane = tid & 63, wave = __builtin_amdgcn_readfirstlane(tid >> 6);
    const int wm = wave / WN, wn = wave % WN;
    const int li = lane & 15, lg = lane >> 4;
    const unsigned lds0 = (unsigned)(size_t)smem;
    const unsigned As = lds0, Bs = lds0 + NS * SA;

    const int Wi = p.Wi;
    struct JobV {
        int nsteps, ntaps, k2, icc2;
        unsigned wofs, wofs2;
        unsigned long long tapcode;
        int Hg, Wg, HWg, npix, tilesN, oh0, ow0, tile0, step0;
        float rcpHW, rcpW;
    };
    auto jobv = [&](int jb) -> JobV {
        if constexpr (TS) {
            (void)jb;
            const int HWg = p.Hg * p.Wg;
            return JobV{p.nsteps, p.ntaps, p.nsteps, p.Ci >> 5, 0u, 0u, p.tapcode, p.Hg, p.Wg, HWg, p.imgs_per_group * HWg, p.tilesN,
                        p.oh0, p.ow0, 0, 0, 1.0f / (float)HWg, 1.0f / (float)p.Wg};
        } else {
            const PconvJob& j = p.job[jb];
            return JobV{j.nsteps, j.ntaps, j.k2, j.icc2, j.wofs, j.wofs2, j.tapcode, j.Hg, j.Wg, j.Hg * j.Wg, j.npix, j.tilesN,
                        j.oh0, j.ow0, j.tile0, j.step0, j.rcpHW, j.rcpW};
        }
    };

    const int nb = gridDim.x, bid = blockIdx.x;
    const int q8 = nb >> 3, r8 = nb & 7, xcd = bid & 7;
    const int rbk = (xcd < r8 ? xcd * (q8 + 1) : r8 * (q8 + 1) + (xcd - r8) * q8) + (bid >> 3);
    const long long S = p.steps_per_block;
    long long w = (long long)rbk * S;
    const long long wend = min(p.total_steps, w + S);

    constexpr unsigned OOB = 0x80000000u;
    const __amdgpu_buffer_rsrc_t rsA = __builtin_amdgcn_make_buffer_rsrc(
        const_cast<unsigned short*>(p.Wsp), 0, TS ? (unsigned)((size_t)p.nsteps * 3 * p.M * 64) : p.wsp_bytes, 0x00020000);
    const __amdgpu_buffer_rsrc_t rsB = __builtin_amdgcn_make_buffer_rsrc(
        const_cast<unsigned char*>(reinterpret_cast<const unsigned char*>(p.Xp) - (size_t)(Wi + 1) * 64), 0,
        (unsigned)(((size_t)(p.Ci >> 5) * 3 * p.xp_pix + (size_t)(Wi + 1)) * 64), 0x00020000);
    const unsigned short* xp2 = TS ? p.Xp : p.Xp2;
    const __amdgpu_buffer_rsrc_t rsB2 = __builtin_amdgcn_make_buffer_rsrc(
        const_cast<unsigned char*>(reinterpret_cast<const unsigned char*>(xp2) - (size_t)(Wi + 1) * 64), 0,
        (unsigned)(((size_t)(p.Ci >> 5) * 3 * p.xp_pix + (size_t)(Wi + 1)) * 64), 0x00020000);
    const int drow = lane >> 2, chunk = (lane & 3) ^ ((lane >> 3) & 3);
    const unsigned fro = li * 64 + ((lg ^ ((li >> 1) & 3)) << 4);
    const unsigned Af0 = As + wm * (16 * FR) * 64 + fro;
    const unsigned Bf0 = Bs + wn * (16 * FC) * 64 + fro;
    unsigned Bfd[3];
#pragma unroll
    for (int d = 0; d < 3; ++d) Bfd[d] = Bs + wn * (16 * FC) * 64 + (li + d) * 64 + ((lg ^ (((li + d) >> 1) & 3)) << 4);
    unsigned Zc[FC];
#pragma unroll
    for (int c = 0; c < FC; ++c) Zc[c] = Bs + (unsigned)((BN + 2 + (li & 7) - 16 * c) * 64 + lg * 16);
    const int ngrpB = (wave + 8 * (RGB - 1) < GB) ? RGB : RGB - 1;
    auto tap_d = [&](int t) { return (int)((unsigned)(p.tapcode >> (4 * t + 2)) & 3u); };

    struct Seg {
        int tile, k0, k1, grp, tn, m0, n0;
        int jb, nsteps, k2, icc2, ntaps;
        unsigned wofs, wofs2;
        unsigned long long tapcode;
        unsigned tstart;
        unsigned voffA, voffB[RGB], vmask[RGB];
        int icc_b, it_b;
        unsigned mLR[FC];
    };
    auto decode = [&](Seg& g) {
        g.jb = 0;
        if constexpr (!TS) {
#pragma unroll
            for (int j = 1; j < PCONV_MAX_JOBS; ++j) g.jb += (int)w >= p.job[j].step0 ? 1 : 0;
        }
        const JobV J = jobv(g.jb);
        const int nsteps = J.nsteps, ntaps = J.ntaps, npix = J.npix, HWg = J.HWg;
        g.nsteps = J.nsteps; g.k2 = J.k2; g.icc2 = J.icc2; g.ntaps = J.ntaps; g.wofs = J.wofs; g.wofs2 = J.wofs2; g.tapcode = J.tapcode;
        const float rcpHW = J.rcpHW, rcpW = J.rcpW;
        const int tiles_pg = p.tilesM * J.tilesN;
        const int tj = (int)((unsigned)(w - J.step0) / (unsigned)nsteps);
        g.k0 = (int)(w - J.step0) - tj * nsteps;
        g.k1 = min(nsteps, g.k0 + (int)(wend - w));
        g.tstart = (unsigned)w - (unsigned)g.k0;
        w += g.k1 - g.k0;
        g.tile = J.tile0 + tj;
        g.grp = tj / tiles_pg;
        const int tl = tj - g.grp * tiles_pg;
        const int tm = p.tn_fast ? tl / J.tilesN : tl % p.tilesM;
        g.tn = p.tn_fast ? tl % J.tilesN : tl / p.tilesM;
        g.m0 = tm * BM; g.n0 = g.tn * BN;
        g.voffA = (unsigned)((g.m0 + drow) * 64 + chunk * 16);
#pragma unroll
        for (int i = 0; i < RGB; ++i) {
            const int n = g.n0 + 16 * (wave + 8 * i) + drow - (TS ? 1 : 0);
            const bool rv = n >= 0 && n < npix && i < ngrpB && (!TS || 16 * (wave + 8 * i) + drow < BN + 2);
            const int nn = rv ? n : 0;
            int img, rem, hg, wg;
            pc_divmod(nn, HWg, rcpHW, img, rem);
            pc_divmod(rem, J.Wg, rcpW, hg, wg);
            const int ih0 = hg * p.sg, iw0 = wg * p.sg;
            unsigned vm = 0;
            if constexpr (TS) {
#pragma unroll
                for (int j = 0; j < 3; ++j) {
                    const int ih = ih0 + (int)((unsigned)(p.tapcode >> (12 * j)) & 3u) - 1;
                    if (rv && (unsigned)ih < (unsigned)p.Hi) vm |= 1u << j;
                }
            } else {
#pragma unroll
                for (int t = 0; t < 9; ++t) {
                    const unsigned f = (unsigned)(J.tapcode >> (4 * t)) & 15u;
                    const int ih = ih0 + (int)(f & 3u) - 1, iw = iw0 + (int)(f >> 2) - 1;
                    if (t < ntaps && rv && (unsigned)ih < (unsigned)p.Hi && (unsigned)iw < (unsigned)Wi) vm |= 1u << t;
                }
            }
            g.vmask[i] = vm;
            g.voffB[i] = (unsigned)((((g.grp * p.imgs_per_group + img) * p.Hi + ih0) * Wi + iw0) * 64 + chunk * 16);
        }
        if constexpr (TS) {
            g.icc_b = g.k0 / 9;
            g.it_b = (g.k0 - g.icc_b * 9) / 3;
#pragma unroll
            for (int c = 0; c < FC; ++c) {
                const int n = g.n0 + wn * (16 * FC) + 16 * c + li;
                int img, rem, hg, wg;
                pc_divmod(n, HWg, rcpHW, img, rem);
                pc_divmod(rem, J.Wg, rcpW, hg, wg);
                const unsigned bl = (unsigned)__builtin_amdgcn_ballot_w64(wg > 0) & 0xffffu;
// ... 245 lines not shown
            for (; s + 3 <= k1; ++s) rstep(std::true_type{}, s);
            for (; s < k1; ++s) rstep(std::false_type{}, s);
        }
#undef PC_READA
#undef PC_READB
#undef PC_LGKM0
#undef PC_LGKM0_COL
        PC_SYNC_LDS();
        PC_T(3);

        const bool more = w < wend;
        Seg nx;
        if (more) {
            decode(nx);
            lead(nx);
        }
        PC_T(4);
        const int tile = cur.tile, grp = cur.grp, tn = cur.tn, m0 = cur.m0, n0 = cur.n0;
        float* fsmem = reinterpret_cast<float*>(smem + NS * SA + NSB * SB);
        bool do_epilogue = true;

        const int nsteps = cur.nsteps;
        if (k0 != 0 || k1 != nsteps) {
            const unsigned t0 = cur.tstart;
            const int b_first = (int)(t0 / (unsigned)S), b_last = (int)((t0 + (unsigned)nsteps - 1u) / (unsigned)S);
            if (rbk != b_first) {
                float* mine = p.slab + (size_t)rbk * 2 * (BM * BN);
#pragma unroll
                for (int r = 0; r < FR; ++r)
#pragma unroll
                    for (int c = 0; c < FC; ++c)
                        *reinterpret_cast<f32x4*>(mine + ((r * FC + c) * 512 + tid) * 4) = acc[r][c];
                pend_tile = tile;
                do_epilogue = false;
            } else {
                int* arrived = reinterpret_cast<int*>(fsmem);
                if (tid == 0) {
                    const int need = b_last - b_first;
                    int got = 0;
                    const int spins = p.lose_part ? (1 << 8) : (1 << 22);
                    for (int it = 0; it < spins && !got; ++it) {
                        got = __hip_atomic_load(p.counters + tile, __ATOMIC_RELAXED, __HIP_MEMORY_SCOPE_AGENT) == need;
                        if (!got) __builtin_amdgcn_s_sleep(4);
                    }
                    if (!got) {
                        if (p.err) __hip_atomic_store(p.err, 1, __ATOMIC_RELAXED, __HIP_MEMORY_SCOPE_AGENT);
                        if (p.err_host) __hip_atomic_store(p.err_host, 1, __ATOMIC_RELAXED, __HIP_MEMORY_SCOPE_SYSTEM);
                    }
                    __hip_atomic_store(p.counters + tile, 0, __ATOMIC_RELAXED, __HIP_MEMORY_SCOPE_AGENT);
                    __builtin_amdgcn_fence(__ATOMIC_ACQUIRE, "agent");
                    asm volatile("s_waitcnt vmcnt(0)" ::: "memory");
                    *arrived = got;
                }
                __syncthreads();
                const float first = *arrived ? 0.f : __builtin_nanf("");
                PC_SYNC_LDS();
#pragma unroll
                for (int r = 0; r < FR; ++r)
#pragma unroll
                    for (int c = 0; c < FC; ++c) acc[r][c] = f32x4{first, first, first, first} + acc[r][c];
                for (int bb = b_first + 1; bb <= b_last; ++bb) {
                    const float* src = p.slab + (size_t)bb * 2 * (BM * BN);
#pragma unroll
                    for (int r = 0; r < FR; r += 2) {
                        f32x4 part[2][FC];
#pragma unroll
                        for (int q = 0; q < 2; ++q)
#pragma unroll
                            for (int c = 0; c < FC; ++c)
                                part[q][c] = *reinterpret_cast<const f32x4*>(src + (((r + q) * FC + c) * 512 + tid) * 4);
#pragma unroll
                        for (int q = 0; q < 2; ++q)
#pragma unroll
                            for (int c = 0; c < FC; ++c) acc[r + q][c] += part[q][c];
                    }
                }
            }
        }

        PC_T(5);
        if (do_epilogue) {
        const int mbase = m0 + wm * (16 * FR) + 4 * lg;
        const JobV J = jobv(cur.jb);
        if (p.stats) {
            float* red = fsmem;
#pragma unroll
            for (int r = 0; r < FR; ++r) {
                f32x4 s1 = {0.f, 0.f, 0.f, 0.f}, s2 = {0.f, 0.f, 0.f, 0.f};
#pragma unroll
                for (int c = 0; c < FC; ++c) {
                    s1 += acc[r][c];
                    s2 += acc[r][c] * acc[r][c];
                }
#pragma unroll
                for (int q = 0; q < 4; ++q) {
                    float u = s1[q], v = s2[q];
                    u += pc_dpp<0xB1>(u); v += pc_dpp<0xB1>(v);
                    u += pc_dpp<0x4E>(u); v += pc_dpp<0x4E>(v);
                    u += pc_dpp<0x12C>(u); v += pc_dpp<0x12C>(v);
                    u += pc_dpp<0x128>(u); v += pc_dpp<0x128>(v);
                    if (li == 0) {
                        const int ml = wm * (16 * FR) + 16 * r + 4 * lg + q;
                        red[(wn * BM + ml) * 2 + 0] = u;
                        red[(wn * BM + ml) * 2 + 1] = v;
                    }
                }
            }
            PC_SYNC_LDS();
            for (int ch = tid; ch < BM; ch += 512) {
                float u = 0.f, v = 0.f;
#pragma unroll
                for (int ww = 0; ww < WN; ++ww) {
                    u += red[(ww * BM + ch) * 2 + 0];
                    v += red[(ww * BM + ch) * 2 + 1];
                }
                float* st = p.stats + (size_t)(grp * J.tilesN + tn) * 2 * p.M;
                st[m0 + ch] = u;
                st[p.M + m0 + ch] = v;
            }
        }
        size_t opix[FC];
        bool ok[FC];
#pragma unroll
        for (int c = 0; c < FC; ++c) {
            const int n = n0 + wn * (16 * FC) + 16 * c + li;
            ok[c] = n < J.npix;
            int img, rem, hg, wg;
            pc_divmod(ok[c] ? n : J.npix - 1, J.HWg, J.rcpHW, img, rem);
            pc_divmod(rem, J.Wg, J.rcpW, hg, wg);
            opix[c] = (size_t)((grp * p.imgs_per_group + img) * p.Ho + hg * p.os + J.oh0) * p.Wo + (wg * p.os + J.ow0);
        }
#pragma unroll
        for (int r = 0; r < FR; r += 2) {
            __builtin_amdgcn_sched_barrier(0);
            const int m = mbase + 16 * r;
            const size_t cb = (size_t)(m0 + wm * (16 * FR) + 16 * r) >> 5;
            f32x4 sc0 = {1.f, 1.f, 1.f, 1.f}, sc1 = sc0, sh0 = {0.f, 0.f, 0.f, 0.f}, sh1 = sh0;
            if (p.scale) {
                sc0 = *reinterpret_cast<const f32x4*>(p.scale + m); sc1 = *reinterpret_cast<const f32x4*>(p.scale + m + 16);
                sh0 = *reinterpret_cast<const f32x4*>(p.shift + m); sh1 = *reinterpret_cast<const f32x4*>(p.shift + m + 16);
            }
#pragma unroll
            for (int c = 0; c < FC; ++c) {
                __builtin_amdgcn_sched_barrier(0);
                const size_t o = opix[c] * p.Co;
                f32x4 v0 = acc[r][c], v1 = acc[r + 1][c];
                if (p.scale) { v0 = v0 * sc0 + sh0; v1 = v1 * sc1 + sh1; }
                if (p.res) {
                    const f32x4 a = *reinterpret_cast<const f32x4*>(p.res + o + m), b = *reinterpret_cast<const f32x4*>(p.res + o + m + 16);
                    v0 += a; v1 += b;
                }
                if (p.resp) {
                    const unsigned char* src = reinterpret_cast<const unsigned char*>(p.resp) + ((cb * 3) * (size_t)p.yp_pix + opix[c]) * 64 + lg * 16;
                    const sp_u32x4 H = *reinterpret_cast<const sp_u32x4*>(src);
                    const sp_u32x4 M = *reinterpret_cast<const sp_u32x4*>(src + (size_t)p.yp_pix * 64);
                    const sp_u32x4 L = *reinterpret_cast<const sp_u32x4*>(src + (size_t)p.yp_pix * 128);
#pragma unroll
                    for (int i = 0; i < 4; ++i) {
                        const float lo = (__builtin_bit_cast(float, H[i] << 16) + __builtin_bit_cast(float, M[i] << 16)) +
                                         __builtin_bit_cast(float, L[i] << 16);
                        const float hi = (__builtin_bit_cast(float, H[i] & 0xffff0000u) + __builtin_bit_cast(float, M[i] & 0xffff0000u)) +
                                         __builtin_bit_cast(float, L[i] & 0xffff0000u);
                        if (i < 2) { v0[2 * i] += lo; v0[2 * i + 1] += hi; }
                        else { v1[2 * (i - 2)] += lo; v1[2 * (i - 2) + 1] += hi; }
                    }
                }
                if (p.relu == 1) {
#pragma unroll
                    for (int q = 0; q < 4; ++q) { v0[q] = fmaxf(v0[q], 0.f); v1[q] = fmaxf(v1[q], 0.f); }
                }
                if (!ok[c]) continue;
                if (p.Y) {
                    *reinterpret_cast<f32x4*>(p.Y + o + m) = v0;
                    *reinterpret_cast<f32x4*>(p.Y + o + m + 16) = v1;
                }
                if (p.Yp) {
                    sp_u32x4 H, M, L;
                    split3(v0, v1, H, M, L);
                    unsigned char* dst = reinterpret_cast<unsigned char*>(p.Yp) + ((cb * 3) * (size_t)p.yp_pix + opix[c]) * 64 + lg * 16;
                    *reinterpret_cast<sp_u32x4*>(dst) = H;
                    *reinterpret_cast<sp_u32x4*>(dst + (size_t)p.yp_pix * 64) = M;
                    *reinterpret_cast<sp_u32x4*>(dst + (size_t)p.yp_pix * 128) = L;
                }
            }
        }
        }
        PC_T(6);
        if (!more) break;
        PC_SYNC_LDS();
        cur = nx;
    }
    if (pend_tile >= 0) {
        asm volatile("s_waitcnt vmcnt(0)" ::: "memory");
        __syncthreads();
        if (tid == 0) {
            __builtin_amdgcn_fence(__ATOMIC_RELEASE, "agent");
            asm volatile("s_waitcnt vmcnt(0)" ::: "memory");
            if (!p.lose_part) __hip_atomic_fetch_add(p.counters + pend_tile, 1, __ATOMIC_RELAXED, __HIP_MEMORY_SCOPE_AGENT);
        }
    }
#undef PC_SYNC_LDS
#ifdef PC_PHASES
    if (tid == 0)
        for (int i = 0; i < 8; ++i) pc_prof[blockIdx.x * 8 + i] = pc_acc[i];
#endif
#endif
}
#ifdef PC_PHASES
extern "C" int fm_debug_pconv_prof(unsigned long long* out)
{
    return (int)hipMemcpyFromSymbol(out, HIP_SYMBOL(pc_prof), sizeof(unsigned long long) * 256 * 8);
}
#endif

__global__ __launch_bounds__(256) void split_weights_bm_kernel(const float* __restrict__ src_base, unsigned short* __restrict__ dst_base,
                                                               const SplitJob* __restrict__ jobs, int njobs)
{
#if __HIP_DEVICE_COMPILE__
    int j = 0;
    while (j + 1 < njobs && (int)blockIdx.x >= jobs[j + 1].blk0) ++j;
    const SplitJob jb = jobs[j];
    const long long idx = (long long)((int)blockIdx.x - jb.blk0) * 256 + threadIdx.x;
    const int nsteps = jb.ntaps * jb.cib;
    if (idx >= (long long)nsteps * jb.M * 4) return;
    const int g = (int)(idx & 3);
    const int m = (int)((idx >> 2) % jb.M);
    const int s = (int)((idx >> 2) / jb.M);
    const int icc = s / jb.ntaps, it = s - icc * jb.ntaps;
    const float* src = (jb.src ? jb.src : src_base + jb.src_off) + ((size_t)m * jb.ntaps + it) * (jb.cib * 32) + icc * 32;
    sp_u32x4 H, M, L;
    split3(ld4(src + 4 * g), ld4(src + 16 + 4 * g), H, M, L);
    unsigned char* dst = reinterpret_cast<unsigned char*>(dst_base + jb.dst_off) + (((size_t)s * 3) * jb.M + m) * 64 + g * 16;
    *reinterpret_cast<sp_u32x4*>(dst) = H;
    *reinterpret_cast<sp_u32x4*>(dst + (size_t)jb.M * 64) = M;
    *reinterpret_cast<sp_u32x4*>(dst + (size_t)jb.M * 128) = L;
#endif
}
void k_split_weights_bm(const float* src_base, unsigned short* dst_base, const SplitJob* jobs, int njobs, int nblocks, hipStream_t s)
{
    if (njobs > 0) hipLaunchKernelGGL(split_weights_bm_kernel, dim3(nblocks), dim3(256), 0, s, src_base, dst_base, jobs, njobs);
}

__global__ __launch_bounds__(256) void split_planes_kernel(const float* __restrict__ x, unsigned short* __restrict__ dst, long long npix,
                                                           int C)
{
#if __HIP_DEVICE_COMPILE__
    const long long idx = (long long)blockIdx.x * 256 + threadIdx.x;
    const int cpp = C >> 3;
    if (idx >= npix * cpp) return;
    const long long pix = idx / cpp;
    const int q = (int)(idx - pix * cpp), cb = q >> 2, g = q & 3;
    const float* src = x + pix * C + cb * 32;
    sp_u32x4 H, M, L;
    split3(ld4(src + 4 * g), ld4(src + 16 + 4 * g), H, M, L);
    unsigned char* d = reinterpret_cast<unsigned char*>(dst) + (((size_t)cb * 3) * npix + pix) * 64 + g * 16;
    *reinterpret_cast<sp_u32x4*>(d) = H;
    *reinterpret_cast<sp_u32x4*>(d + (size_t)npix * 64) = M;
    *reinterpret_cast<sp_u32x4*>(d + (size_t)npix * 128) = L;
#endif
}
void k_split_planes(const float* x, unsigned short* dst, long long npix, int C, hipStream_t s)
{
    const long long n = npix * (C >> 3);
    if (n > 0) hipLaunchKernelGGL(split_planes_kernel, dim3((unsigned)((n + 255) / 256)), dim3(256), 0, s, x, dst, npix, C);
}

int pconv_max_blocks() { return 256; }
static int g_lose_part = 0;
void pconv_debug_lose_part(int on) { g_lose_part = on; }
size_t pconv_slab_floats() { return (size_t)pconv_max_blocks() * 2 * 128 * 256; }
int pconv_tile_m(int M) { return M >= 128 ? 128 : 64; }
int pconv_tile_n(int M) { (void)M; return 256; }
bool pconv_takes(int M, int Ci, long long xp_pix, int Wi)
{
    if (M % 64 != 0 || (M > 64 && M % 128 != 0) || Ci % 32 != 0) return false;
    return ((long long)(Ci >> 5) * 3 * xp_pix + Wi + 1) * 64 < 0x7ff00000LL && xp_pix < (1LL << 22);
}

bool pconv_uses_ts(const IgemmParams& p)
{
    bool ts = p.njobs == 0 && p.ntaps == 9 && p.sg == 1 && p.Hg == p.Hi && p.Wg == p.Wi;
    for (int j = 0; ts && j < 3; ++j) {
        ts = p.dh[3 * j] == p.dh[3 * j + 1] && p.dh[3 * j] == p.dh[3 * j + 2];
        int seen = 0;
        for (int k = 0; k < 3; ++k) seen |= 1 << (p.dw[3 * j + k] + 1);
        ts = ts && seen == 7;
    }
    return ts;
}

void launch_pconv(IgemmParams p, int groups, hipStream_t s)
{
    static bool attr_done = false;
    constexpr int LDS_L = 2 * 3 * (128 + 256) * 64 + 4 * 128 * 2 * 4;
    constexpr int LDS_S = 2 * 3 * (64 + 256) * 64 + 4 * 128 * 2 * 4;
    constexpr int LDS_LT = 2 * 3 * 128 * 64 + 2 * 3 * 272 * 64 + 4 * 128 * 2 * 4;
    constexpr int LDS_ST = 2 * 3 * 64 * 64 + 2 * 3 * 272 * 64 + 4 * 128 * 2 * 4;
    if (!attr_done) {
        set_max_dyn_lds(reinterpret_cast<const void*>(&pconv_kernel<4, 4, 2, 6, true>), LDS_LT, "pconv_kernel<4, 4, 2, 6, true>");
        set_max_dyn_lds(reinterpret_cast<const void*>(&pconv_kernel<4, 4, 2, 9, true>), LDS_LT, "pconv_kernel<4, 4, 2, 9, true>");
        set_max_dyn_lds(reinterpret_cast<const void*>(&pconv_kernel<2, 4, 2, 6, true>), LDS_ST, "pconv_kernel<2, 4, 2, 6, true>");
        set_max_dyn_lds(reinterpret_cast<const void*>(&pconv_kernel<2, 4, 2, 9, true>), LDS_ST, "pconv_kernel<2, 4, 2, 9, true>");
        set_max_dyn_lds(reinterpret_cast<const void*>(&pconv_kernel<4, 4, 2, 6>), LDS_L, "pconv_kernel<4, 4, 2, 6>");
        set_max_dyn_lds(reinterpret_cast<const void*>(&pconv_kernel<4, 4, 2, 9>), LDS_L, "pconv_kernel<4, 4, 2, 9>");
        set_max_dyn_lds(reinterpret_cast<const void*>(&pconv_kernel<2, 4, 2, 6>), LDS_S, "pconv_kernel<2, 4, 2, 6>");
        set_max_dyn_lds(reinterpret_cast<const void*>(&pconv_kernel<2, 4, 2, 9>), LDS_S, "pconv_kernel<2, 4, 2, 9>");
        attr_done = true;
    }
    const bool ts = pconv_uses_ts(p);
    p.tapcode = pconv_tapcode(p.dh, p.dw, p.ntaps);
    if (p.njobs == 0) {
        p.njobs = 1;
        PconvJob& j = p.job[0];
        j.ntaps = p.ntaps; j.tapcode = p.tapcode;
        j.cib = j.icc2 = p.Ci >> 5; j.wofs = j.wofs2 = 0;
        j.Hg = p.Hg; j.Wg = p.Wg; j.oh0 = p.oh0; j.ow0 = p.ow0;
    }
    if (!p.Xp2) p.Xp2 = p.Xp;
    long long T = 0;
    p.total_steps = 0; p.nsteps = 0; p.wsp_bytes = 0;
    for (int k = 0; k < p.njobs; ++k) {
        PconvJob& j = p.job[k];
        j.nsteps = j.ntaps * j.cib; j.k2 = j.ntaps * j.icc2;
        j.npix = p.imgs_per_group * j.Hg * j.Wg;
        j.rcpHW = 1.0f / (float)(j.Hg * j.Wg); j.rcpW = 1.0f / (float)j.Wg;
        j.tilesN = (j.npix + 255) / 256;
        j.tile0 = (int)T; j.step0 = (int)p.total_steps;
        T += (long long)p.tilesM * j.tilesN * groups;
        p.total_steps += (long long)p.tilesM * j.tilesN * groups * j.nsteps;
        p.nsteps = std::max(p.nsteps, j.nsteps);
        const long long step_bytes = 3LL * p.M * 64;
        p.wsp_bytes = (unsigned)std::max<long long>(p.wsp_bytes, std::max(j.wofs + j.k2 * step_bytes, j.wofs2 + (j.nsteps - j.k2) * step_bytes));
        j.wofs2 -= (unsigned)(j.k2 * step_bytes);
    }
    for (int k = p.njobs; k < PCONV_MAX_JOBS; ++k) p.job[k].step0 = 0x7fffffff;
    p.tn_fast = p.tilesM > 1 && (long long)p.M * p.nsteps * 192 > (3LL << 20);
    static const int forced = getenv("FM_IGEMM_BLOCKS") ? atoi(getenv("FM_IGEMM_BLOCKS")) : 0;
    int nblk = p.total_steps >= 4LL * pconv_max_blocks() ? pconv_max_blocks() : (int)std::min<long long>(pconv_max_blocks(), T);
    if (forced > 0) nblk = (int)std::min<long long>(std::min(forced, pconv_max_blocks()), p.total_steps);
    p.steps_per_block = (int)((p.total_steps + nblk - 1) / nblk);
    if (forced <= 0 && p.steps_per_block > p.nsteps / 2 && (long long)p.nsteps * 128 * 192 > (2LL << 20)) {
        for (int P = 1; P <= 12; ++P) {
            if (p.nsteps % P) continue;
            const int q = p.nsteps / P;
            const int sq = (p.steps_per_block + q - 1) / q * q;
            if ((long long)sq * 100 <= (long long)p.steps_per_block * 102) { p.steps_per_block = sq; break; }
        }
    }
    dim3 grid(nblk);
    p.lose_part = g_lose_part ? 1 : 0;
    if (ts) {
        if (p.M >= 128) {
            if (p.sp == 9) hipLaunchKernelGGL((pconv_kernel<4, 4, 2, 9, true>), grid, dim3(512), LDS_LT, s, p);
            else hipLaunchKernelGGL((pconv_kernel<4, 4, 2, 6, true>), grid, dim3(512), LDS_LT, s, p);
        } else {
            if (p.sp == 9) hipLaunchKernelGGL((pconv_kernel<2, 4, 2, 9, true>), grid, dim3(512), LDS_ST, s, p);
            else hipLaunchKernelGGL((pconv_kernel<2, 4, 2, 6, true>), grid, dim3(512), LDS_ST, s, p);
        }
        return;
    }
    if (p.M >= 128) {
        if (p.sp == 9) hipLaunchKernelGGL((pconv_kernel<4, 4, 2, 9>), grid, dim3(512), LDS_L, s, p);
        else hipLaunchKernelGGL((pconv_kernel<4, 4, 2, 6>), grid, dim3(512), LDS_L, s, p);
    } else {
        if (p.sp == 9) hipLaunchKernelGGL((pconv_kernel<2, 4, 2, 9>), grid, dim3(512), LDS_S, s, p);
        else hipLaunchKernelGGL((pconv_kernel<2, 4, 2, 6>), grid, dim3(512), LDS_S, s, p);
    }
}

__global__ __launch_bounds__(256) void planes_to_f32_kernel(const unsigned short* __restrict__ src, float* __restrict__ x, long long npix, int C)
{
#if __HIP_DEVICE_COMPILE__
    const long long idx = (long long)blockIdx.x * 256 + threadIdx.x;
    const int cpp = C >> 3;
    if (idx >= npix * cpp) return;
    const long long pix = idx / cpp;
    const int q = (int)(idx - pix * cpp), cb = q >> 2, g = q & 3;
    const unsigned char* s = reinterpret_cast<const unsigned char*>(src) + (((size_t)cb * 3) * npix + pix) * 64 + g * 16;
    const sp_u32x4 H = *reinterpret_cast<const sp_u32x4*>(s);
    const sp_u32x4 M = *reinterpret_cast<const sp_u32x4*>(s + (size_t)npix * 64);
    const sp_u32x4 L = *reinterpret_cast<const sp_u32x4*>(s + (size_t)npix * 128);
    float v[8];
#pragma unroll
    for (int i = 0; i < 4; ++i) {
        v[2 * i] = (__builtin_bit_cast(float, H[i] << 16) + __builtin_bit_cast(float, M[i] << 16)) + __builtin_bit_cast(float, L[i] << 16);
        v[2 * i + 1] = (__builtin_bit_cast(float, H[i] & 0xffff0000u) + __builtin_bit_cast(float, M[i] & 0xffff0000u)) +
                       __builtin_bit_cast(float, L[i] & 0xffff0000u);
    }
    float* d = x + pix * C + cb * 32;
    *reinterpret_cast<f32x4*>(d + 4 * g) = f32x4{v[0], v[1], v[2], v[3]};
    *reinterpret_cast<f32x4*>(d + 16 + 4 * g) = f32x4{v[4], v[5], v[6], v[7]};
#endif
}
void k_planes_to_f32(const unsigned short* src, float* x, long long npix, int C, hipStream_t s)
{
    const long long n = npix * (C >> 3);
    if (n > 0) hipLaunchKernelGGL(planes_to_f32_kernel, dim3((unsigned)((n + 255) / 256)), dim3(256), 0, s, src, x, npix, C);
}
```

### fedmlp_amd/engine.py

```python
import ctypes as C

import numpy as np
import torch

from . import _lib, spec

MODEL_IDS = {"Resnet18": 0, "Efficient_b0": 1}
PRECISION_IDS = {"fp32": 0, "bf16": 1}
PRODUCT_FORMS = {None: 0, 6: 3, 0: 1, 9: 2}


def _ptr(t):
    if t is None:
        return None
    assert t.is_cuda and t.is_contiguous() and t.dtype in (torch.float32, torch.int32, torch.bfloat16), \
        (t.device, t.dtype, t.is_contiguous())
    return C.c_void_p(t.data_ptr())


def _cargs(args):
    return [_ptr(a) if torch.is_tensor(a) else a for a in args]


class RoflHeads:
# ... 662 lines not shown
        _lib.check(self.lib.fm_profile_ops(self.h, int(enable), buf, (1 << 16) if read else 0))
        rows = []
        if read:
            for line in buf.value.decode().splitlines():
                lab, n, ms = line.split("\t")
                rows.append((lab, int(n), float(ms)))
        return rows

    def debug_conv_info(self, conv):
        info = (C.c_int32 * 16)()
        _lib.check(self.lib.fm_debug_conv_info(self.h, conv, info))
        keys = ("cin", "cout", "k", "stride", "pad", "hin", "win", "hout", "wout", "cin_p", "Kw", "kw_p", "cout_p")
        return dict(zip(keys, list(info)))

    def debug_stem_masks(self, imgs, groups):
        H2, W2 = self.in_h // 2, self.in_w // 2
        bits = np.empty((imgs, H2, W2, 8), np.uint8)
        code = np.empty((imgs, H2 // 2, W2 // 2, 64), np.uint8)
        _lib.check(self.lib.fm_debug_stem_masks(self.h, imgs, groups, bits.ctypes.data_as(C.c_void_p),
                                                code.ctypes.data_as(C.c_void_p)))
        return np.unpackbits(bits, axis=-1, bitorder="little").astype(bool), code

    def debug_get_grads(self):
        flat = np.empty(self.nf, np.float32)
        _lib.check(self.lib.fm_debug_get_grads(self.h, flat.ctypes.data_as(C.c_void_p)))
        return flat

    WAIT_KINDS = ("side_begin", "side_guard", "side_join", "ev_in", "ev_t")

    def debug_lane_delay(self, lane, at, micros):
        _lib.check(self.lib.fm_debug_lane_delay(self.h, int(lane), int(at), int(micros)))

    def debug_lane_points(self, disarm=False):
        o = (C.c_int64 * 16)()
        _lib.check(self.lib.fm_debug_lane_points(self.h, o, int(bool(disarm))))
        n = len(self.WAIT_KINDS)
        return {"points": (int(o[0]), int(o[1])), "fired": bool(o[2]),
                "waits": {k: int(o[3 + i]) for i, k in enumerate(self.WAIT_KINDS)},
                "skipped": {k: int(o[3 + n + i]) for i, k in enumerate(self.WAIT_KINDS)}}

    def debug_drop_wait(self, kind, on=True):
        which = self.WAIT_KINDS.index(kind) if isinstance(kind, str) else int(kind)
        _lib.check(self.lib.fm_debug_drop_wait(self.h, which, int(bool(on))))

    def debug_optim_arena(self, which):
        p, n = C.c_void_p(), C.c_int64()
        _lib.check(self.lib.fm_debug_optim_arena(self.h, int(which), C.byref(p), C.byref(n)))
        return _device_view(p.value, n.value, self.device)

    def debug_entry_spans(self):
        n = len(spec.entries(self.model, self.n_classes))
        a = np.empty((n, 2), np.int64)
        _lib.check(self.lib.fm_debug_entry_spans(self.h, a.ctypes.data_as(C.c_void_p), n))
        return a

    def debug_pw(self, op, conv, x, dy, out, imgs, groups=1, psc=None, psh=None, gate=None, stats=None):
        self._enqueue()
        _lib.check(self.lib.fm_debug_pw(self.h, op, conv, _ptr(x), _ptr(dy), _ptr(out), imgs, groups, _ptr(psc),
                                        _ptr(psh), _ptr(gate), _ptr(stats)))

    def debug_pw_fwd(self, conv, x, out, imgs, groups=1, scale=None, shift=None, res=None, act=0, psc=None, psh=None, gate=None,
                     stats=None):
        self._enqueue()
        _lib.check(self.lib.fm_debug_pw_fwd(self.h, conv, _ptr(x), _ptr(out), imgs, groups, _ptr(scale), _ptr(shift), _ptr(res),
                                            int(act), _ptr(psc), _ptr(psh), _ptr(gate), _ptr(stats)))

    def debug_proj_bwd(self, conv, phase, dyp, yd, bn, gate, ds, imgs, groups, out, pool5=None):
        self._enqueue()
        _lib.check(self.lib.fm_debug_proj_bwd(self.h, conv, phase, _ptr(dyp), _ptr(yd), _ptr(bn), _ptr(gate), _ptr(ds), imgs,
                                              groups, _ptr(out), _ptr(pool5)))

    def debug_exp_bwd(self, conv, da, ye, x, res, bn, imgs, groups, dx, dw):
        self._enqueue()
        _lib.check(self.lib.fm_debug_exp_bwd(self.h, conv, _ptr(da), _ptr(ye), _ptr(x), _ptr(res), _ptr(bn), imgs, groups,
                                             _ptr(dx), _ptr(dw)))

    def debug_activation(self, kind, block, imgs):
        dims = (C.c_int32 * 4)()
        _lib.check(self.lib.fm_debug_activation(self.h, kind, block, imgs, None, dims))
        out = np.empty(tuple(dims), np.float32)
        _lib.check(self.lib.fm_debug_activation(self.h, kind, block, imgs, out.ctypes.data_as(C.c_void_p), dims))
        return np.ascontiguousarray(out.transpose(0, 3, 1, 2))

    def debug_num_convs(self):
        return self.lib.fm_debug_num_convs(self.h)

    def debug_conv(self, op, conv, x, dy, out, imgs, groups=1, stats=None):
        self._enqueue()
        _lib.check(self.lib.fm_debug_conv(self.h, op, conv, _ptr(x), _ptr(dy), _ptr(out), imgs, groups,
                                          _ptr(stats)))

    def debug_conv_fwd(self, conv, x, out, imgs, groups=1, scale=None, shift=None, res=None, act=0, psc=None, psh=None,
                       gate=None, stats=None):
        self._enqueue()
        _lib.check(self.lib.fm_debug_conv_fwd(self.h, conv, _ptr(x), _ptr(out), imgs, groups, _ptr(scale), _ptr(shift),
                                              _ptr(res), int(act), _ptr(psc), _ptr(psh), _ptr(gate), _ptr(stats)))

    def debug_conv_planes(self, conv, xp, imgs, scale, shift, res=None, resp=None, relu=0, out=None, outp=None):
        def words(t):
            assert t is None or (t.is_cuda and t.is_contiguous() and t.dtype == torch.int16), "planes are int16 device tensors"
            return None if t is None else C.c_void_p(t.data_ptr())
        self._enqueue()
        _lib.check(self.lib.fm_debug_conv_planes(self.h, conv, words(xp), imgs, _ptr(scale), _ptr(shift), _ptr(res), words(resp),
                                                 int(relu), _ptr(out), words(outp)))

    CONV_ARMS = ("igemm", "igemm_stem", "stem_rows", "pconv_ts", "pconv_tap", "pwgrad", "pwgrad_ring", "wgrad_generic",
                 "wgrad_skinny", "stem_dgrad")

    def debug_conv_arm(self, op, conv, imgs):
        rc = self.lib.fm_debug_conv_arm(self.h, op, conv, imgs)
        if rc < 0:
            _lib.check(rc)
        return self.CONV_ARMS[rc]

    def debug_block_dgrad(self, block, dy1, dyd, dx, imgs):
        self._enqueue()
        _lib.check(self.lib.fm_debug_block_dgrad(self.h, block, _ptr(dy1), _ptr(dyd), _ptr(dx), imgs))

    EW_OPS = ("split_planes", "planes_to_f32", "bn_finalize", "bn_finalize_frozen", "bn_eval_affine", "bn_apply",
              "bn_apply_planes", "stem_pool", "stem_pool_planes", "stem_pool_bwd", "stem_pool_bn_reduce", "stem_pool_bn_apply",
              "bn_bwd_reduce", "bn_bwd_finalize", "bn_bwd_apply", "bn_bwd_apply_planes")

    def debug_ew(self, op, ptrs, dims, scalars=()):
        assert len(ptrs) <= 12 and len(dims) <= 5 and len(scalars) <= 2, (len(ptrs), len(dims), len(scalars))
        for t in ptrs:
            assert t is None or (t.is_cuda and t.is_contiguous()), op
        p = (C.c_void_p * 12)(*[None if t is None else t.data_ptr() for t in ptrs])
        d = (C.c_int32 * 5)(*[int(v) for v in dims])
        _lib.check(self.lib.fm_debug_ew(self.h, self.EW_OPS.index(op), p, d, _lib.fvec(list(scalars) + [0.0] * (2 - len(scalars)))))

    EFF_OPS = ("dw_fwd", "dw_dgrad", "dw_wgrad", "se_fwd", "se_scale", "se_bwd_bn1", "se_wgrad", "bnact_apply", "chan_reduce",
               "bnact_bwd_apply")

    def debug_eff_ws(self, op, dims):
        assert len(dims) <= 13, len(dims)
        d = (C.c_int32 * 13)(*[int(v) for v in dims])
        n = (C.c_int64 * 4)()
        _lib.check(self.lib.fm_debug_eff_ws(self.EFF_OPS.index(op), d, n))
        return list(n)

    def debug_eff(self, op, ptrs, dims, scalars=()):
        assert len(ptrs) <= 15 and len(dims) <= 13 and len(scalars) <= 1, (len(ptrs), len(dims), len(scalars))
        for t in ptrs:
            assert t is None or (t.is_cuda and t.is_contiguous()), op
        served = C.c_int32(-1)
        p = (C.c_void_p * 16)(*([None if t is None else t.data_ptr() for t in ptrs] + [None] * (15 - len(ptrs))
                                + [C.addressof(served)]))
        d = (C.c_int32 * 13)(*[int(v) for v in dims])
        _lib.check(self.lib.fm_debug_eff(self.h, self.EFF_OPS.index(op), p, d, _lib.fvec(list(scalars) + [0.0] * (1 - len(scalars)))))
        return served.value == 1

    HEAD_OPS = ("avgpool", "fc_fwd", "fc_bwd", "loss_bce", "loss_stage1", "loss_stage2", "loss_fixmatch")

    def debug_head(self, op, ptrs, dims, scalars=()):
        assert len(ptrs) <= 8 and len(dims) <= 5 and len(scalars) <= 2, (len(ptrs), len(dims), len(scalars))
        keep, raw = [], []
        for t in ptrs:
            if t is None:
                raw.append(None)
            elif isinstance(t, (list, tuple)):
                keep.append(_lib.fvec(t))
                raw.append(C.addressof(keep[-1]))
            else:
                assert t.is_cuda and t.is_contiguous(), op
                raw.append(t.data_ptr())
        p = (C.c_void_p * 8)(*(raw + [None] * (8 - len(raw))))
        d = (C.c_int32 * 5)(*[int(v) for v in dims])
        _lib.check(self.lib.fm_debug_head(self.h, self.HEAD_OPS.index(op), p, d, _lib.fvec(list(scalars) + [0.0] * (2 - len(scalars)))))


class _CudaArrayView:

    def __init__(self, ptr, n):
        self.__cuda_array_interface__ = {"shape": (n,), "typestr": "<f4", "data": (ptr, False),
                                         "version": 2, "strides": None}


def _device_view(ptr, n, device):
    return torch.as_tensor(_CudaArrayView(ptr, n), device=device)


_ENGINES = {}


def get_engine(model, n_classes, in_h, in_w, max_images, device=None, precision="fp32"):
    if device is None:
        from .launch import default_device
        device = default_device()
    key = (model, int(n_classes), int(in_h), int(in_w), str(device), precision)
    e = _ENGINES.get(key)
    if e is None or e.max_images < max_images:
        if e is not None:
            owner = getattr(e, "_owner", None)
            if owner is not None:
                owner._pull()
                owner._engine = None
            e._owner = None
            e.close()
        e = Engine(model, n_classes, in_h, in_w, max_images, device, precision)
        _ENGINES[key] = e
# ... 13 lines not shown
```

### include/fedmlp_hip_debug.h

```cpp
#ifndef FEDMLP_HIP_DEBUG_H
#define FEDMLP_HIP_DEBUG_H

#include "fedmlp_hip.h"

#ifdef __cplusplus
extern "C" {
#endif

int fm_debug_conv_info(fm_engine* e, int32_t conv, int32_t* info16);
int fm_debug_num_convs(fm_engine* e);
int fm_debug_conv(fm_engine* e, int32_t op, int32_t conv, const float* x_dev, const float* dy_dev,
                  float* out_dev, int32_t imgs, int32_t groups, float* stats_dev);

int fm_debug_conv_fwd(fm_engine* e, int32_t conv, const float* x_dev, float* out_dev, int32_t imgs, int32_t groups,
                      const float* scale_dev, const float* shift_dev, const float* res_dev, int32_t act, const float* psc_dev,
                      const float* psh_dev, const float* gate_dev, float* stats_dev);

int fm_debug_conv_planes(fm_engine* e, int32_t conv, const uint16_t* xp_dev, int32_t imgs, const float* scale_dev,
                         const float* shift_dev, const float* res_dev, const uint16_t* resp_dev, int32_t relu, float* out_dev,
                         uint16_t* outp_dev);

enum { FM_ARM_IGEMM = 0, FM_ARM_IGEMM_STEM, FM_ARM_STEM_ROWS, FM_ARM_PCONV_TS, FM_ARM_PCONV_TAP, FM_ARM_PWGRAD, FM_ARM_PWGRAD_RING,
       FM_ARM_WGRAD_GENERIC, FM_ARM_WGRAD_SKINNY, FM_ARM_STEM_DGRAD };
int fm_debug_conv_arm(fm_engine* e, int32_t op, int32_t conv, int32_t imgs);

int fm_debug_block_dgrad(fm_engine* e, int32_t block, const float* dy1_dev, const float* dyd_dev, float* dx_dev, int32_t imgs);

int fm_debug_pw(fm_engine* e, int32_t op, int32_t conv, const void* x_dev, const void* dy_dev, void* out_dev,
                int32_t imgs, int32_t groups, const float* psc_dev, const float* psh_dev, const float* gate_dev,
                float* stats_dev);

int fm_debug_pw_fwd(fm_engine* e, int32_t conv, const void* x_dev, void* out_dev, int32_t imgs, int32_t groups,
                    const float* scale_dev, const float* shift_dev, const void* res_dev, int32_t act, const float* psc_dev,
                    const float* psh_dev, const float* gate_dev, float* stats_dev);

int fm_debug_proj_bwd(fm_engine* e, int32_t conv, int32_t phase, const void* dyp_dev, const void* yd_dev, const float* bn_dev,
                      const float* gate_dev, const float* ds_dev, int32_t imgs, int32_t groups, void* out_dev,
                      float* pool5_dev);

int fm_debug_exp_bwd(fm_engine* e, int32_t conv, const void* da_dev, const void* ye_dev, const void* x_dev, const void* res_dev,
                     const float* bn_dev, int32_t imgs, int32_t groups, void* dx_dev, float* dw_dev);

int fm_debug_activation(fm_engine* e, int32_t kind, int32_t block, int32_t imgs, float* host_nhwc,
                        int32_t* dims4);

int fm_debug_stem_masks(fm_engine* e, int32_t imgs, int32_t groups, uint8_t* relu_bits_host, uint8_t* argmax_host);

int fm_debug_lose_part(int32_t on);

enum { FM_WAIT_SIDE_BEGIN = 0, FM_WAIT_SIDE_GUARD, FM_WAIT_SIDE_JOIN, FM_WAIT_EV_IN, FM_WAIT_EV_T };
#define FM_WAIT_KINDS 5
#define FM_LANE_DELAY_MAX_US 20000
int fm_debug_lane_delay(fm_engine* e, int32_t lane, int64_t at, int32_t micros);
int fm_debug_lane_points(fm_engine* e, int64_t* out16, int32_t disarm);
int fm_debug_drop_wait(fm_engine* e, int32_t which, int32_t on);

int fm_debug_get_grads(fm_engine* e, float* host_f32);
int fm_debug_optim_arena(fm_engine* e, int32_t which, float** dev_ptr, int64_t* numel);
int fm_debug_entry_spans(fm_engine* e, int64_t* off_len, int32_t n_entries);

enum {
    FM_EW_SPLIT_PLANES = 0, FM_EW_PLANES_TO_F32, FM_EW_BN_FINALIZE, FM_EW_BN_FINALIZE_FROZEN, FM_EW_BN_EVAL_AFFINE, FM_EW_BN_APPLY,
    FM_EW_BN_APPLY_PLANES, FM_EW_STEM_POOL, FM_EW_STEM_POOL_PLANES, FM_EW_STEM_POOL_BWD, FM_EW_STEM_POOL_BN_REDUCE,
    FM_EW_STEM_POOL_BN_APPLY, FM_EW_BN_BWD_REDUCE, FM_EW_BN_BWD_FINALIZE, FM_EW_BN_BWD_APPLY, FM_EW_BN_BWD_APPLY_PLANES
};
#define FM_EW_NPTR 12
#define FM_EW_NDIM 5
#define FM_EW_NSCAL 2
int fm_debug_ew(fm_engine* e, int32_t op, void* const* p, const int32_t* d, const float* sc);

enum { FM_EFF_DW_FWD = 0, FM_EFF_DW_DGRAD, FM_EFF_DW_WGRAD, FM_EFF_SE_FWD, FM_EFF_SE_SCALE, FM_EFF_SE_BWD_BN1, FM_EFF_SE_WGRAD,
       FM_EFF_BNACT_APPLY, FM_EFF_CHAN_REDUCE, FM_EFF_BNACT_BWD_APPLY };
#define FM_EFF_NPTR 16
#define FM_EFF_NDIM 13
#define FM_EFF_NWS 4
int fm_debug_eff(fm_engine* e, int32_t op, void* const* p, const int32_t* d, const float* sc);
int fm_debug_eff_ws(int32_t op, const int32_t* d, int64_t* floats);

enum { FM_HD_AVGPOOL = 0, FM_HD_FC_FWD, FM_HD_FC_BWD, FM_HD_LOSS_BCE, FM_HD_LOSS_STAGE1, FM_HD_LOSS_STAGE2, FM_HD_LOSS_FIXMATCH };
#define FM_HD_NPTR 8
#define FM_HD_NDIM 5
#define FM_HD_NSCAL 2
int fm_debug_head(fm_engine* e, int32_t op, void* const* p, const int32_t* d, const float* sc);

#ifdef __cplusplus
}
#endif
#endif
```

Before: 6238 images/sec.

## Fuse BatchNorm-backward reduction sums into the conv2 data-gradient epilogue

In each ResNet-18 basic block, the c2 data-gradient convolution (planes tap-sharing kernel) now computes the per-channel BatchNorm-backward partial sums for bn1 in its epilogue, reading the saved bn1 output y to rebuild the ReLU mask. The separate k_bn_bwd_reduce pass over dz is then skipped, and finalize reads the per-tile partials. This removes one full read of the gradient and activation tensors per block. The cost is extra y loads and an LDS reduction in the conv epilogue, which may raise register pressure. The workspace partial buffer grows, and a new template variant plus debug entry points are added.

```diff
diff --git a/fedmlp_amd/_lib.py b/fedmlp_amd/_lib.py
--- a/fedmlp_amd/_lib.py
+++ b/fedmlp_amd/_lib.py
@@ -123,6 +123,8 @@
     "fm_debug_conv": (C.c_int, [_P, _I32, _I32, _P, _P, _P, _I32, _I32, _P]),
     "fm_debug_conv_fwd": (C.c_int, [_P, _I32, _P, _P, _I32, _I32, _P, _P, _P, _I32, _P, _P, _P, _P]),
     "fm_debug_block_dgrad": (C.c_int, [_P, _I32, _P, _P, _P, _I32]),
+    "fm_debug_conv_dgrad_bn": (C.c_int, [_P, _I32, _P, _P, _P, _P, _P, _P, _I32, _I32, _I32, _P, _P]),
+    "fm_debug_bn_bwd_fused": (C.c_int, [_P, _I32, _I32, _I32, _I32]),
     "fm_debug_conv_planes": (C.c_int, [_P, _I32, _P, _I32, _P, _P, _P, _P, _I32, _P, _P]),
     "fm_debug_conv_arm": (C.c_int, [_P, _I32, _I32, _I32]),
     "fm_debug_pw": (C.c_int, [_P, _I32, _I32, _P, _P, _P, _I32, _I32, _P, _P, _P, _P]),
@@ -133,6 +135,7 @@
     "fm_debug_optim_arena": (C.c_int, [_P, _I32, C.POINTER(_P), C.POINTER(_I64)]),
     "fm_debug_entry_spans": (C.c_int, [_P, _P, _I32]),
     "fm_debug_activation": (C.c_int, [_P, _I32, _I32, _I32, _P, C.POINTER(_I32)]),
+    "fm_debug_bn_group_stats": (C.c_int, [_P, _I32, _I32, _P]),
     "fm_debug_stem_masks": (C.c_int, [_P, _I32, _I32, _P, _P]),
     "fm_debug_lose_part": (C.c_int, [_I32]),
     "fm_debug_lane_delay": (C.c_int, [_P, _I32, _I64, _I32]),
diff --git a/fedmlp_amd/csrc/common.h b/fedmlp_amd/csrc/common.h
--- a/fedmlp_amd/csrc/common.h
+++ b/fedmlp_amd/csrc/common.h
@@ -150,7 +150,15 @@
     PconvJob job[PCONV_MAX_JOBS];
     const unsigned short* Xp2 = nullptr;
     unsigned wsp_bytes = 0;
-};
+    const float* bs_y = nullptr;
+    const float* bs_scale = nullptr;
+    const float* bs_shift = nullptr;
+    const float* bs_mean = nullptr;
+    const float* bs_istd = nullptr;
+    float* bs_part = nullptr;
+    unsigned bs_y_bytes = 0;
+};
+bool pconv_takes_bn_sums(const IgemmParams& p, int groups);
 void pconv_debug_lose_part(int on);
 
 struct WgradParams {
diff --git a/fedmlp_amd/csrc/engine.hip b/fedmlp_amd/csrc/engine.hip
--- a/fedmlp_amd/csrc/engine.hip
+++ b/fedmlp_amd/csrc/engine.hip
@@ -217,6 +217,7 @@
     uint8_t* idx0 = nullptr;
     float *GA = nullptr, *GB = nullptr, *GE = nullptr;
     float *ws_stats = nullptr, *ws_part = nullptr;
+    size_t ws_part_floats = 0;
     int stats_conv = -1, stats_tiles_n = 0;
     size_t slab_floats = 0;
     float *ca = nullptr, *cb = nullptr, *cc = nullptr;
@@ -879,7 +880,14 @@
         DALLOC(e->hfeat, B * e->D);
     }
     DALLOC(e->ws_stats, max_stats);
-    DALLOC(e->ws_part, (size_t)2 * (1024 + 32) * 2 * e->maxC);
+    e->ws_part_floats = (size_t)2 * (1024 + 32) * 2 * e->maxC;
+    if (e->model == 0)
+        for (const Block& k : e->blocks) {
+            const Conv& c = e->convs[k.c1];
+            const size_t tiles = (B * c.hout * c.wout + pconv_tile_n(c.cout_p) - 1) / pconv_tile_n(c.cout_p) + 2;
+            e->ws_part_floats = std::max(e->ws_part_floats, (tiles + 2 * 32) * 2 * c.cout_p);
+        }
+    DALLOC(e->ws_part, e->ws_part_floats);
     e->slab_floats = std::max<size_t>(max_slab * 8, (size_t)48 << 20);
     DALLOC(e->main.ws_slab, e->slab_floats);
     e->main.rec = e->main.ws_slab;
@@ -1188,11 +1196,28 @@
 }
 
 struct DgradAdd { const float* res = nullptr; bool acc_cls0 = false; };
-void conv_dgrad(fm_engine* e, Lane& L, int ci, In dy, float* dx, int imgs, const DgradAdd& add = {})
+struct DgradSums { const float *y = nullptr, *mask_scale = nullptr, *mask_shift = nullptr, *mean = nullptr, *istd = nullptr;
+                   float* part = nullptr; int groups = 1; };
+static int dgrad_sums_tiles(const Conv& c, int imgs_per_group)
+{
+    return (imgs_per_group * c.hin * c.win + pconv_tile_n(c.cin_p) - 1) / pconv_tile_n(c.cin_p);
+}
+static bool dgrad_takes_sums(const fm_engine* e, const Conv& c, int imgs, int groups, size_t part_floats)
+{
+    if (!e->planes || (e->products != 6 && e->products != 9) || groups < 1 || imgs % groups != 0 || c.ncls != 1) return false;
+    if (dgrad_arm(e, c, imgs) != Arm::PconvTs) return false;
+    return (size_t)groups * (dgrad_sums_tiles(c, imgs / groups) + 32) * 2 * c.cin_p <= part_floats;
+}
+void conv_dgrad(fm_engine* e, Lane& L, int ci, In dy, float* dx, int imgs, const DgradAdd& add = {}, const DgradSums& sums = {})
 {
     Conv& c = e->convs[ci];
     const Arm arm = dgrad_arm(e, c, imgs);
     const long long xp_pix = (long long)imgs * c.hout * c.wout;
+    const int groups = sums.groups;
+    if ((sums.part || groups != 1) && (arm != Arm::PconvTs || c.ncls != 1 || add.res || add.acc_cls0 || groups < 1 || imgs % groups != 0)) {
+        soft(e, hipErrorInvalidValue);
+        return;
+    }
     switch (arm) {
     case Arm::PwConv: {
         PwParams q{};
@@ -1219,16 +1244,21 @@
         p.res = add.res ? add.res : ((add.acc_cls0 && d.ph == 0 && d.pw == 0) ? dx : nullptr);
         p.Ho = c.hin; p.Wo = c.win; p.Co = c.cin_p;
         p.os = c.stride; p.oh0 = d.ph; p.ow0 = d.pw;
-        p.imgs_per_group = imgs;
+        p.imgs_per_group = imgs / groups;
         p.relu = 0;
         const int bn = planes ? pconv_tile_n(c.cin_p) : igemm_tile_n(c.cin_p);
-        p.tilesN = (imgs * p.Hg * p.Wg + bn - 1) / bn;
+        p.tilesN = (p.imgs_per_group * p.Hg * p.Wg + bn - 1) / bn;
         const double flops = 2.0 * c.macs_per_img * imgs * d.taps.n / (double)(c.k * c.k);
         if (planes) {
             p.Xp = dy.p; p.xp_pix = xp_pix; p.Wsp = e->wpl_d + d.pl_off;
             p.tilesM = c.cin_p / pconv_tile_m(c.cin_p);
+            if (sums.part) {
+                p.bs_y = sums.y; p.bs_scale = sums.mask_scale; p.bs_shift = sums.mask_shift; p.bs_mean = sums.mean; p.bs_istd = sums.istd;
+                p.bs_part = sums.part;
+                if (!pconv_takes_bn_sums(p, groups)) { soft(e, hipErrorInvalidValue); return; }
+            }
             ProfScope ps(e, L, prof_family(pconv_arm(p), c.cin_p), flops);
-            launch_pconv(p, 1, L.st);
+            launch_pconv(p, groups, L.st);
         } else {
             p.W = d.wpack; p.X = dy.f; p.zeros = e->zeros; p.nsteps = d.nsteps;
             if (!e->planes && d.pl_off >= 0) p.Wsp = e->wpl_d + d.pl_off;
@@ -1412,7 +1442,7 @@
 }
 enum class Mask { None, Z, ZPlane, OwnOutput };
 void bn_bwd(fm_engine* e, Lane& L, int bi, const float* dz, Out dy, int groups, int imgs_per_group, bool frozen, Mask mask = Mask::None,
-            In z = {}, float* dyh_out = nullptr)
+            In z = {}, float* dyh_out = nullptr, int sums_tiles = 0)
 {
     const Conv& c = e->convs[bi];
     Bn& b = e->bns[bi];
@@ -1424,8 +1454,9 @@
     if (mask == Mask::Z || (mask == Mask::OwnOutput && !from_y && z.f)) zf = z.f;
     else if (mask == Mask::ZPlane) zh = z.p;
     else if (mask == Mask::OwnOutput) { msc = b.scale; msh = b.shift; }
-    k_bn_bwd_reduce(dz, zf, c.y, b.mean, b.istd, e->ws_part, groups, pix, b.C, L.st, msc, msh, zh);
-    bn_bwd_finalize(e, L, b, groups, bn_bwd_blocks(pix), pix, frozen);
+    if (sums_tiles > 0 && mask != Mask::OwnOutput) { soft(e, hipErrorInvalidValue); return; }
+    if (sums_tiles <= 0) k_bn_bwd_reduce(dz, zf, c.y, b.mean, b.istd, e->ws_part, groups, pix, b.C, L.st, msc, msh, zh);
+    bn_bwd_finalize(e, L, b, groups, sums_tiles > 0 ? sums_tiles : bn_bwd_blocks(pix), pix, frozen);
     if (dy.p) k_bn_bwd_apply_planes(dz, zf, c.y, e->ca, e->cb, e->cc, dy.f, dy.p, dyh_out, groups, pix, b.C, L.st, msc, msh, zh);
     else k_bn_bwd_apply(dz, zf, c.y, e->ca, e->cb, e->cc, dy.f, dyh_out, groups, pix, b.C, L.st, msc, msh);
 }
@@ -1812,6 +1843,15 @@
     side_end(e, k, par);
 }
 
+static bool bn_bwd_fused(const fm_engine* e, const Block& blk, int imgs, int groups, bool frozen)
+{
+    const char* fu = getenv("FM_BN_BWD_FUSED");
+    if ((fu && atoi(fu) == 0) || frozen || e->model != 0) return false;
+    const Conv &c1 = e->convs[blk.c1], &c2 = e->convs[blk.c2];
+    if (c2.cin_p != c1.cout_p || c2.hin != c1.hout || c2.win != c1.wout) return false;
+    return dgrad_takes_sums(e, c2, imgs, groups, e->ws_part_floats);
+}
+
 void backward_and_step(fm_engine* e, int groups, int B, const Bwd& bw)
 {
     const int imgs = groups * B;
@@ -1853,10 +1893,17 @@
         { OP(L, "bn_bwd"); bn_bwd(e, L, blk.c2, ga, dy2, groups, B, bw.frozen, zo.f ? Mask::Z : Mask::ZPlane, zo, ga); }
         if (blk.ds >= 0) { side_guard(e, 1, par); OP(L, "bn_bwd"); bn_bwd(e, L, blk.ds, ga, dyd, groups, B, bw.frozen); }
         side_guard(e, 2, par);
-        { OP(L, "conv_dgrad"); conv_dgrad(e, L, blk.c2, dy2, g.dy1.f, imgs); }
+        const bool fused = bn_bwd_fused(e, blk, imgs, groups, bw.frozen);
+        const Bn& b1 = e->bns[blk.c1];
+        { OP(L, "conv_dgrad");
+          if (fused) conv_dgrad(e, L, blk.c2, dy2, g.dy1.f, imgs, {},
+                                {.y = e->convs[blk.c1].y, .mask_scale = b1.scale, .mask_shift = b1.shift, .mean = b1.mean, .istd = b1.istd,
+                                 .part = e->ws_part, .groups = groups});
+          else conv_dgrad(e, L, blk.c2, dy2, g.dy1.f, imgs); }
         if (conv_on(e, tr, blk.c2))
             side_wgrad(e, forked, 0, par, "conv_wgrad", [&](Lane& SL) { conv_wgrad(e, SL, blk.c2, kept(a.z1), dy2, imgs); });
-        { OP(L, "bn_bwd"); bn_bwd(e, L, blk.c1, g.dy1.f, dy1, groups, B, bw.frozen, Mask::OwnOutput, kept(a.z1)); }
+        { OP(L, "bn_bwd"); bn_bwd(e, L, blk.c1, g.dy1.f, dy1, groups, B, bw.frozen, Mask::OwnOutput, kept(a.z1), nullptr,
+                                  fused ? dgrad_sums_tiles(e->convs[blk.c2], B) : 0); }
         { OP(L, "conv_dgrad");
           if (blk.ds < 0) conv_dgrad(e, L, blk.c1, dy1, ge, imgs, {.res = ga});
           else if (!block_dgrad(e, L, blk.c1, blk.ds, dy1, dyd, ge, imgs)) {
@@ -3771,11 +3818,20 @@
 int fm_debug_activation(fm_engine* e, int32_t kind, int32_t block, int32_t imgs, float* host_nhwc, int32_t* dims4)
 {
     ARGCHK(e && dims4 && e->model == 0, "ResNet-18 engine only");
-    ARGCHK(block >= 0 && block < (int)e->blocks.size() && (kind == 0 || kind == 1), "kind/block");
+    ARGCHK(block >= 0 && block < (int)e->blocks.size() && kind >= 0 && kind <= 3, "kind/block");
     ARGCHK(imgs >= 1 && imgs <= e->maxB, "imgs");
-    const Out t = kind == 0 ? e->acts.blk[block].z1 : e->acts.blk[block].out;
     const Conv& c = e->convs[e->blocks[block].c1];
     dims4[0] = imgs; dims4[1] = c.hout; dims4[2] = c.wout; dims4[3] = c.cout;
+    if (kind >= 2) {
+        ARGCHK(kind == 2 || block < 2, "d z1 is kept for blocks 0 and 1 only");
+        const float* src = kind == 2 ? c.y : e->rg[block & 1].dy1.f;
+        if (host_nhwc) {
+            HIPCHK(hipMemcpyAsync(host_nhwc, src, (size_t)imgs * c.hout * c.wout * c.cout * 4, hipMemcpyDeviceToHost, e->main.st));
+            HIPCHK(hipStreamSynchronize(e->main.st));
+        }
+        return FM_OK;
+    }
+    const Out t = kind == 0 ? e->acts.blk[block].z1 : e->acts.blk[block].out;
     if (host_nhwc) {
         if (e->planes && (kind == 0 || block + 1 < (int)e->blocks.size()))
             k_planes_to_f32(t.p, t.f, (long long)imgs * c.hout * c.wout, c.cout, e->main.st);
@@ -3783,6 +3839,18 @@
                               hipMemcpyDeviceToHost, e->main.st));
         HIPCHK(hipStreamSynchronize(e->main.st));
     }
+    return FM_OK;
+}
+
+int fm_debug_bn_group_stats(fm_engine* e, int32_t block, int32_t groups, float* host4)
+{
+    ARGCHK(e && host4 && e->model == 0 && block >= 0 && block < (int)e->blocks.size(), "a ResNet-18 engine and a block index");
+    ARGCHK(groups >= 1 && groups <= 2, "groups");
+    const Bn& b = e->bns[e->blocks[block].c1];
+    const float* src[4] = {b.mean, b.istd, b.scale, b.shift};
+    for (int k = 0; k < 4; ++k)
+        HIPCHK(hipMemcpyAsync(host4 + (size_t)k * groups * b.C, src[k], (size_t)groups * b.C * 4, hipMemcpyDeviceToHost, e->main.st));
+    HIPCHK(hipStreamSynchronize(e->main.st));
     return FM_OK;
 }
 
@@ -3876,6 +3944,53 @@
         conv_dgrad(e, e->main, blk.c1, {dy1_dev}, dx_dev, imgs, {.acc_cls0 = true});
     }
     return FM_OK;
+}
+
+int fm_debug_conv_dgrad_bn(fm_engine* e, int32_t conv, const float* dy_dev, const float* y_dev, const float* mask_scale_dev,
+                           const float* mask_shift_dev, const float* mean_dev, const float* istd_dev, int32_t imgs, int32_t groups,
+                           int32_t fused, float* dz_dev, float* sums_dev)
+{
+    ARGCHK(e && conv >= 0 && conv < (int)e->convs.size(), "conv index");
+    ARGCHK(dy_dev && y_dev && mask_scale_dev && mask_shift_dev && mean_dev && istd_dev && dz_dev && sums_dev, "null tensor");
+    ARGCHK(e->model == 0 && !e->precision && e->planes, "fm_debug_conv_dgrad_bn: a planes-mode precision-0 ResNet-18 engine");
+    ARGCHK(imgs >= 1 && imgs <= e->maxB && groups >= 1 && imgs % groups == 0, "imgs / groups");
+    Conv& c = e->convs[conv];
+    ARGCHK(dgrad_takes_sums(e, c, imgs, groups, e->ws_part_floats),
+           "the data gradient with BatchNorm-backward sums: a 3x3 stride-1 convolution on a 6- or 9-product planes handle");
+    ARGCHK((size_t)imgs * c.hout * c.wout * c.cout_p * 3 <= e->xp_scratch_elems, "dy outside the planes scratch");
+    ensure_packed(e);
+    const int B = imgs / groups, C = c.cin_p, pix = B * c.hin * c.win;
+    int tiles;
+    if (fused) {
+        tiles = dgrad_sums_tiles(c, B);
+        conv_dgrad(e, e->main, conv, {dy_dev}, dz_dev, imgs, {},
+                   {.y = y_dev, .mask_scale = mask_scale_dev, .mask_shift = mask_shift_dev, .mean = mean_dev, .istd = istd_dev,
+                    .part = e->ws_part, .groups = groups});
+    } else {
+        tiles = bn_bwd_blocks(pix);
+        conv_dgrad(e, e->main, conv, {dy_dev}, dz_dev, imgs, {}, {.groups = groups});
+        k_bn_bwd_reduce(dz_dev, nullptr, y_dev, mean_dev, istd_dev, e->ws_part, groups, pix, C, e->main.st, mask_scale_dev, mask_shift_dev,
+                        nullptr);
+    }
+    std::vector<float> h((size_t)groups * tiles * 2 * C), o((size_t)groups * 2 * C, 0.f);
+    HIPCHK(hipMemcpyAsync(h.data(), e->ws_part, h.size() * 4, hipMemcpyDeviceToHost, e->main.st));
+    HIPCHK(hipStreamSynchronize(e->main.st));
+    STEP_DONE(e);
+    for (int g = 0; g < groups; ++g)
+        for (int k = 0; k < 2 * C; ++k) {
+            double sum = 0;
+            for (int t = 0; t < tiles; ++t) sum += h[((size_t)g * tiles + t) * 2 * C + k];
+            o[(size_t)g * 2 * C + k] = (float)sum;
+        }
+    HIPCHK(hipMemcpy(sums_dev, o.data(), o.size() * 4, hipMemcpyHostToDevice));
+    return FM_OK;
+}
+
+int fm_debug_bn_bwd_fused(fm_engine* e, int32_t block, int32_t imgs, int32_t groups, int32_t frozen)
+{
+    ARGCHK(e && e->model == 0 && block >= 0 && block < (int)e->blocks.size(), "a ResNet-18 engine and a block index");
+    ARGCHK(imgs >= 1 && imgs <= e->maxB && groups >= 1 && imgs % groups == 0, "imgs / groups");
+    return bn_bwd_fused(e, e->blocks[block], imgs, groups, frozen != 0) ? 1 : 0;
 }
 
 int fm_debug_conv_info(fm_engine* e, int32_t conv, int32_t* info16)
diff --git a/fedmlp_amd/csrc/pconv.hip b/fedmlp_amd/csrc/pconv.hip
--- a/fedmlp_amd/csrc/pconv.hip
+++ b/fedmlp_amd/csrc/pconv.hip
@@ -45,10 +45,11 @@
 #ifndef PC_WAVES_PER_EU
 #define PC_WAVES_PER_EU 2
 #endif
-template <int FR, int FC, int NS, int SP, bool TS = false>
+template <int FR, int FC, int NS, int SP, bool TS = false, bool BS = false>
 __global__ __launch_bounds__(512, PC_WAVES_PER_EU) void pconv_kernel(const IgemmParams p)
 {
 #if __HIP_DEVICE_COMPILE__
+    static_assert(!BS || TS, "BatchNorm-backward sums: the tap-row-sharing form only");
 #ifdef PC_PHASES
     unsigned long long pc_acc[8] = {0, 0, 0, 0, 0, 0, 0, 0};
     unsigned long long pc_t = clock64();
@@ -110,6 +111,7 @@
     const __amdgpu_buffer_rsrc_t rsB2 = __builtin_amdgcn_make_buffer_rsrc(
         const_cast<unsigned char*>(reinterpret_cast<const unsigned char*>(xp2) - (size_t)(Wi + 1) * 64), 0,
         (unsigned)(((size_t)(p.Ci >> 5) * 3 * p.xp_pix + (size_t)(Wi + 1)) * 64), 0x00020000);
+    const __amdgpu_buffer_rsrc_t rsY = __builtin_amdgcn_make_buffer_rsrc(const_cast<float*>(BS ? p.bs_y : nullptr), 0, BS ? p.bs_y_bytes : 0u, 0x00020000);
     const int drow = lane >> 2, chunk = (lane & 3) ^ ((lane >> 3) & 3);
     const unsigned fro = li * 64 + ((lg ^ ((li >> 1) & 3)) << 4);
     const unsigned Af0 = As + wm * (16 * FR) * 64 + fro;
@@ -521,7 +523,7 @@
         if (do_epilogue) {
         const int mbase = m0 + wm * (16 * FR) + 4 * lg;
         const JobV J = jobv(cur.jb);
-        if (p.stats) {
+        if (!BS && p.stats) {
             float* red = fsmem;
 #pragma unroll
             for (int r = 0; r < FR; ++r) {
@@ -569,27 +571,71 @@
             pc_divmod(rem, J.Wg, J.rcpW, hg, wg);
             opix[c] = (size_t)((grp * p.imgs_per_group + img) * p.Ho + hg * p.os + J.oh0) * p.Wo + (wg * p.os + J.ow0);
         }
+        f32x4 by0[BS ? FC : 1], by1[BS ? FC : 1];
+        auto load_y = [&](int r) {
+#pragma unroll
+            for (int c = 0; c < FC; ++c) {
+                const unsigned o = ((unsigned)opix[c] * (unsigned)p.Co + (unsigned)(mbase + 16 * r)) * 4u;
+                by0[BS ? c : 0] = __builtin_bit_cast(f32x4, __builtin_amdgcn_raw_buffer_load_b128(rsY, o, 0, 0));
+                by1[BS ? c : 0] = __builtin_bit_cast(f32x4, __builtin_amdgcn_raw_buffer_load_b128(rsY, o + 64u, 0, 0));
+            }
+        };
+        if constexpr (BS) load_y(0);
 #pragma unroll
         for (int r = 0; r < FR; r += 2) {
             __builtin_amdgcn_sched_barrier(0);
             const int m = mbase + 16 * r;
             const size_t cb = (size_t)(m0 + wm * (16 * FR) + 16 * r) >> 5;
             f32x4 sc0 = {1.f, 1.f, 1.f, 1.f}, sc1 = sc0, sh0 = {0.f, 0.f, 0.f, 0.f}, sh1 = sh0;
-            if (p.scale) {
+            if (!BS && p.scale) {
                 sc0 = *reinterpret_cast<const f32x4*>(p.scale + m); sc1 = *reinterpret_cast<const f32x4*>(p.scale + m + 16);
                 sh0 = *reinterpret_cast<const f32x4*>(p.shift + m); sh1 = *reinterpret_cast<const f32x4*>(p.shift + m + 16);
+            }
+            if constexpr (BS) {
+                float* red = fsmem;
+#pragma unroll
+                for (int h = 0; h < 2; ++h) {
+                    const size_t gm = (size_t)grp * p.M + m + 16 * h;
+                    const f32x4 bsc = *reinterpret_cast<const f32x4*>(p.bs_scale + gm), bsh = *reinterpret_cast<const f32x4*>(p.bs_shift + gm);
+                    const f32x4 bmu = *reinterpret_cast<const f32x4*>(p.bs_mean + gm), bis = *reinterpret_cast<const f32x4*>(p.bs_istd + gm);
+                    f32x4 s1 = {0.f, 0.f, 0.f, 0.f}, s2 = {0.f, 0.f, 0.f, 0.f};
+#pragma unroll
+                    for (int c = 0; c < FC; ++c) {
+                        const f32x4 yy = h ? by1[c] : by0[c];
+                        f32x4 d = acc[r + h][c];
+#pragma unroll
+                        for (int q = 0; q < 4; ++q) d[q] = (ok[c] && __builtin_fmaf(yy[q], bsc[q], bsh[q]) > 0.f) ? d[q] : 0.f;
+                        const f32x4 xh = (yy - bmu) * bis;
+                        s1 += d;
+                        s2 += d * xh;
+                    }
+#pragma unroll
+                    for (int q = 0; q < 4; ++q) {
+                        float u = s1[q], v = s2[q];
+                        u += pc_dpp<0xB1>(u); v += pc_dpp<0xB1>(v);
+                        u += pc_dpp<0x4E>(u); v += pc_dpp<0x4E>(v);
+                        u += pc_dpp<0x12C>(u); v += pc_dpp<0x12C>(v);
+                        u += pc_dpp<0x128>(u); v += pc_dpp<0x128>(v);
+                        if (li == 0) {
+                            const int ml = wm * (16 * FR) + 16 * (r + h) + 4 * lg + q;
+                            red[(wn * BM + ml) * 2 + 0] = u;
+                            red[(wn * BM + ml) * 2 + 1] = v;
+                        }
+                    }
+                }
+                if (r + 2 < FR) load_y(r + 2);
             }
 #pragma unroll
             for (int c = 0; c < FC; ++c) {
                 __builtin_amdgcn_sched_barrier(0);
                 const size_t o = opix[c] * p.Co;
                 f32x4 v0 = acc[r][c], v1 = acc[r + 1][c];
-                if (p.scale) { v0 = v0 * sc0 + sh0; v1 = v1 * sc1 + sh1; }
-                if (p.res) {
+                if (!BS && p.scale) { v0 = v0 * sc0 + sh0; v1 = v1 * sc1 + sh1; }
+                if (!BS && p.res) {
                     const f32x4 a = *reinterpret_cast<const f32x4*>(p.res + o + m), b = *reinterpret_cast<const f32x4*>(p.res + o + m + 16);
                     v0 += a; v1 += b;
                 }
-                if (p.resp) {
+                if (!BS && p.resp) {
                     const unsigned char* src = reinterpret_cast<const unsigned char*>(p.resp) + ((cb * 3) * (size_t)p.yp_pix + opix[c]) * 64 + lg * 16;
                     const sp_u32x4 H = *reinterpret_cast<const sp_u32x4*>(src);
                     const sp_u32x4 M = *reinterpret_cast<const sp_u32x4*>(src + (size_t)p.yp_pix * 64);
@@ -604,7 +650,7 @@
                         else { v1[2 * (i - 2)] += lo; v1[2 * (i - 2) + 1] += hi; }
                     }
                 }
-                if (p.relu == 1) {
+                if (!BS && p.relu == 1) {
 #pragma unroll
                     for (int q = 0; q < 4; ++q) { v0[q] = fmaxf(v0[q], 0.f); v1[q] = fmaxf(v1[q], 0.f); }
                 }
@@ -613,7 +659,7 @@
                     *reinterpret_cast<f32x4*>(p.Y + o + m) = v0;
                     *reinterpret_cast<f32x4*>(p.Y + o + m + 16) = v1;
                 }
-                if (p.Yp) {
+                if (!BS && p.Yp) {
                     sp_u32x4 H, M, L;
                     split3(v0, v1, H, M, L);
                     unsigned char* dst = reinterpret_cast<unsigned char*>(p.Yp) + ((cb * 3) * (size_t)p.yp_pix + opix[c]) * 64 + lg * 16;
@@ -621,6 +667,21 @@
                     *reinterpret_cast<sp_u32x4*>(dst + (size_t)p.yp_pix * 64) = M;
                     *reinterpret_cast<sp_u32x4*>(dst + (size_t)p.yp_pix * 128) = L;
                 }
+            }
+        }
+        if constexpr (BS) {
+            const float* red = fsmem;
+            PC_SYNC_LDS();
+            for (int ch = tid; ch < BM; ch += 512) {
+                float u = 0.f, v = 0.f;
+#pragma unroll
+                for (int ww = 0; ww < WN; ++ww) {
+                    u += red[(ww * BM + ch) * 2 + 0];
+                    v += red[(ww * BM + ch) * 2 + 1];
+                }
+                float* st = p.bs_part + (size_t)(grp * J.tilesN + tn) * 2 * p.M;
+                st[m0 + ch] = u;
+                st[p.M + m0 + ch] = v;
             }
         }
         }
@@ -728,6 +789,14 @@
     return ts;
 }
 
+bool pconv_takes_bn_sums(const IgemmParams& p, int groups)
+{
+    const long long ybytes = (long long)groups * p.imgs_per_group * p.Ho * p.Wo * p.Co * 4;
+    return pconv_uses_ts(p) && p.bs_part && p.bs_y && p.bs_scale && p.bs_shift && p.bs_mean && p.bs_istd && p.Y && !p.Yp && !p.res &&
+           !p.resp && !p.scale && !p.stats && !p.relu && p.os == 1 && p.oh0 == 0 && p.ow0 == 0 && p.Ho == p.Hg && p.Wo == p.Wg &&
+           p.Co == p.M && (p.sp == 6 || p.sp == 9) && groups >= 1 && ybytes < 0x7ff00000LL;
+}
+
 void launch_pconv(IgemmParams p, int groups, hipStream_t s)
 {
     static bool attr_done = false;
@@ -740,6 +809,10 @@
         set_max_dyn_lds(reinterpret_cast<const void*>(&pconv_kernel<4, 4, 2, 9, true>), LDS_LT, "pconv_kernel<4, 4, 2, 9, true>");
         set_max_dyn_lds(reinterpret_cast<const void*>(&pconv_kernel<2, 4, 2, 6, true>), LDS_ST, "pconv_kernel<2, 4, 2, 6, true>");
         set_max_dyn_lds(reinterpret_cast<const void*>(&pconv_kernel<2, 4, 2, 9, true>), LDS_ST, "pconv_kernel<2, 4, 2, 9, true>");
+        set_max_dyn_lds(reinterpret_cast<const void*>(&pconv_kernel<4, 4, 2, 6, true, true>), LDS_LT, "pconv_kernel<4, 4, 2, 6, true, true>");
+        set_max_dyn_lds(reinterpret_cast<const void*>(&pconv_kernel<4, 4, 2, 9, true, true>), LDS_LT, "pconv_kernel<4, 4, 2, 9, true, true>");
+        set_max_dyn_lds(reinterpret_cast<const void*>(&pconv_kernel<2, 4, 2, 6, true, true>), LDS_ST, "pconv_kernel<2, 4, 2, 6, true, true>");
+        set_max_dyn_lds(reinterpret_cast<const void*>(&pconv_kernel<2, 4, 2, 9, true, true>), LDS_ST, "pconv_kernel<2, 4, 2, 9, true, true>");
         set_max_dyn_lds(reinterpret_cast<const void*>(&pconv_kernel<4, 4, 2, 6>), LDS_L, "pconv_kernel<4, 4, 2, 6>");
         set_max_dyn_lds(reinterpret_cast<const void*>(&pconv_kernel<4, 4, 2, 9>), LDS_L, "pconv_kernel<4, 4, 2, 9>");
         set_max_dyn_lds(reinterpret_cast<const void*>(&pconv_kernel<2, 4, 2, 6>), LDS_S, "pconv_kernel<2, 4, 2, 6>");
@@ -747,6 +820,9 @@
         attr_done = true;
     }
     const bool ts = pconv_uses_ts(p);
+    const bool bs = p.bs_part != nullptr;
+    if (bs && !pconv_takes_bn_sums(p, groups)) return;
+    if (bs) p.bs_y_bytes = (unsigned)((long long)groups * p.imgs_per_group * p.Ho * p.Wo * p.Co * 4);
     p.tapcode = pconv_tapcode(p.dh, p.dw, p.ntaps);
     if (p.njobs == 0) {
         p.njobs = 1;
@@ -788,6 +864,16 @@
     }
     dim3 grid(nblk);
     p.lose_part = g_lose_part ? 1 : 0;
+    if (bs) {
+        if (p.M >= 128) {
+            if (p.sp == 9) hipLaunchKernelGGL((pconv_kernel<4, 4, 2, 9, true, true>), grid, dim3(512), LDS_LT, s, p);
+            else hipLaunchKernelGGL((pconv_kernel<4, 4, 2, 6, true, true>), grid, dim3(512), LDS_LT, s, p);
+        } else {
+            if (p.sp == 9) hipLaunchKernelGGL((pconv_kernel<2, 4, 2, 9, true, true>), grid, dim3(512), LDS_ST, s, p);
+            else hipLaunchKernelGGL((pconv_kernel<2, 4, 2, 6, true, true>), grid, dim3(512), LDS_ST, s, p);
+        }
+        return;
+    }
     if (ts) {
         if (p.M >= 128) {
             if (p.sp == 9) hipLaunchKernelGGL((pconv_kernel<4, 4, 2, 9, true>), grid, dim3(512), LDS_LT, s, p);
diff --git a/fedmlp_amd/engine.py b/fedmlp_amd/engine.py
--- a/fedmlp_amd/engine.py
+++ b/fedmlp_amd/engine.py
@@ -768,6 +768,16 @@
         _lib.check(self.lib.fm_debug_activation(self.h, kind, block, imgs, out.ctypes.data_as(C.c_void_p), dims))
         return np.ascontiguousarray(out.transpose(0, 3, 1, 2))
 
+    def debug_bn1_group_stats(self, block, groups):
+        Cc = self.debug_conv_info(self._bn1_conv(block))["cout"]
+        out = np.empty((4, groups, Cc), np.float32)
+        _lib.check(self.lib.fm_debug_bn_group_stats(self.h, block, groups, out.ctypes.data_as(C.c_void_p)))
+        return out
+
+    @staticmethod
+    def _bn1_conv(block):
+        return 1 + 2 * block + sum(1 for b in (2, 4, 6) if b < block)
+
     def debug_num_convs(self):
         return self.lib.fm_debug_num_convs(self.h)
 
@@ -802,6 +812,17 @@
     def debug_block_dgrad(self, block, dy1, dyd, dx, imgs):
         self._enqueue()
         _lib.check(self.lib.fm_debug_block_dgrad(self.h, block, _ptr(dy1), _ptr(dyd), _ptr(dx), imgs))
+
+    def debug_conv_dgrad_bn(self, conv, dy, y, mask_scale, mask_shift, mean, istd, imgs, groups, dz, sums, fused=True):
+        self._enqueue()
+        _lib.check(self.lib.fm_debug_conv_dgrad_bn(self.h, conv, _ptr(dy), _ptr(y), _ptr(mask_scale), _ptr(mask_shift), _ptr(mean),
+                                                   _ptr(istd), imgs, groups, int(bool(fused)), _ptr(dz), _ptr(sums)))
+
+    def debug_bn_bwd_fused(self, block, imgs, groups, frozen=False):
+        rc = self.lib.fm_debug_bn_bwd_fused(self.h, block, imgs, groups, int(bool(frozen)))
+        if rc < 0:
+            _lib.check(rc)
+        return bool(rc)
 
     EW_OPS = ("split_planes", "planes_to_f32", "bn_finalize", "bn_finalize_frozen", "bn_eval_affine", "bn_apply",
               "bn_apply_planes", "stem_pool", "stem_pool_planes", "stem_pool_bwd", "stem_pool_bn_reduce", "stem_pool_bn_apply",
diff --git a/include/fedmlp_hip_debug.h b/include/fedmlp_hip_debug.h
--- a/include/fedmlp_hip_debug.h
+++ b/include/fedmlp_hip_debug.h
@@ -26,6 +26,11 @@
 
 int fm_debug_block_dgrad(fm_engine* e, int32_t block, const float* dy1_dev, const float* dyd_dev, float* dx_dev, int32_t imgs);
 
+int fm_debug_conv_dgrad_bn(fm_engine* e, int32_t conv, const float* dy_dev, const float* y_dev, const float* mask_scale_dev,
+                           const float* mask_shift_dev, const float* mean_dev, const float* istd_dev, int32_t imgs, int32_t groups,
+                           int32_t fused, float* dz_dev, float* sums_dev);
+int fm_debug_bn_bwd_fused(fm_engine* e, int32_t block, int32_t imgs, int32_t groups, int32_t frozen);
+
 int fm_debug_pw(fm_engine* e, int32_t op, int32_t conv, const void* x_dev, const void* dy_dev, void* out_dev,
                 int32_t imgs, int32_t groups, const float* psc_dev, const float* psh_dev, const float* gate_dev,
                 float* stats_dev);
@@ -43,6 +48,7 @@
 
 int fm_debug_activation(fm_engine* e, int32_t kind, int32_t block, int32_t imgs, float* host_nhwc,
                         int32_t* dims4);
+int fm_debug_bn_group_stats(fm_engine* e, int32_t block, int32_t groups, float* host4);
 
 int fm_debug_stem_masks(fm_engine* e, int32_t imgs, int32_t groups, uint8_t* relu_bits_host, uint8_t* argmax_host);
 
```

Result: no change. 6235 images/sec, median of 2 (-0.0%).
